# fogg-lab/tissue-model-analysis-tools

Measured on AMD Instinct MI355X. Metric: images/sec (1024x1024 uint16) through compute_branches, higher is better.
Workload: dtype f32; 1 GPU; 256 synthetic 1024x1024 uint16 Z-projections per GPU (256 distinct), inputs pre-resident in HBM (host-pointer entry adds 2 MB/image of H2D), tiled UNet seg (200 patches/image, random-init structured weights) + DMT branch extraction, default_branching_computation.json; images_per_gpu=256, distinct_images=256, patches_per_image=200, rows_gathered=256

## Files before the change

### include/tmat.h

```cpp
#ifndef TMAT_H
#define TMAT_H
#include <stddef.h>
#include <stdint.h>

#ifdef __cplusplus
extern "C" {
#endif

typedef struct tmat_ctx *tmat_handle;

#define TMAT_OK 0
#define TMAT_E_ARG (-1)
#define TMAT_E_HIP (-2)
#define TMAT_E_WEIGHTS (-3)
#define TMAT_E_CAP (-4)

const char *tmat_last_error(void);
int tmat_version(void);

int tmat_create(int device_id, const void *weights_blob, size_t n_bytes, int max_patches, tmat_handle *out);
int tmat_create_plain(int device_id, tmat_handle *out);
void tmat_destroy(tmat_handle h);
int tmat_sync(tmat_handle h);

// ... 288 lines not shown
#define TMAT_PRECISION_F32 0
#define TMAT_PRECISION_BF16X3 1
#define TMAT_PRECISION_BF16X6 2
int tmat_set_precision(tmat_handle h, int mode);

int tmat_set_input_norm(tmat_handle h, int on, double norm_mean, double norm_std);

int tmat_prof_enable(tmat_handle h, int on);
int tmat_prof_read(tmat_handle h, double *ms, int64_t *launches, double *flops, int reset);

int tmat_debug_poison(tmat_handle h, int byte_pattern);

int tmat_debug_held_bytes(tmat_handle h, size_t *device_bytes, size_t *pinned_bytes);

int tmat_debug_filter_stages(tmat_handle h, const uint8_t *mask, int n, int hh, int ww, int use_median, int remove_isolated, uint8_t *median,
                             int32_t *labels, int32_t *stats, uint8_t *skeleton, uint8_t *filtered, int32_t *thin_launches);

int tmat_roi_plan(int hh, int ww, int patch, int n_up, const int *channels, int max_classes, int tiles_cap, int *tiles_per_img,
                  int *n_classes, int *tile_class, int *tile_rank, int *class_count, int *rects, double *mac_planned, double *mac_full);

int tmat_roi_plan_tight(int hh, int ww, int patch, int n_up, const int *channels, int max_classes, int tiles_cap, int *tiles_per_img,
                        int *n_classes, int *tile_class, int *tile_rank, int *class_count, int *rects, double *mac_planned, double *mac_full);
int tmat_roi_plan_exact(int hh, int ww, int patch, int n_up, const int *channels, int max_classes, int tiles_cap, int *tiles_per_img,
                        int *n_classes, int *tile_class, int *tile_rank, int *class_count, int *rects, double *mac_planned, double *mac_full);

int tmat_roi_plan_down(int hh, int ww, int patch, int n_up, const int *up_channels, int n_down, const int *down_channels,
                       unsigned fused_mask, int max_classes, int *n_classes, int *rects, int *needs, double *mac_planned,
                       double *mac_full, double *bytes_planned, double *bytes_full, int *free_tile);

int tmat_roi_sep_tiles(int hh, int ww, int patch, int n_up, const int *up_channels, int n_down, const int *down_channels,
                       unsigned fused_mask, int layer, int k, int cap, int *n_tiles, int *n_full, int *tiles);

int tmat_roi_plan_const(int hh, int ww, int patch, int n_up, const int *up_channels, int n_down, const int *down_channels,
                        unsigned fused_mask, int max_classes, int *n_classes, int *nonconst, int *live, int *rect_live, int *fill,
                        int *stored, double *mac_live, double *bytes_live);
int tmat_roi_sep_tiles_live(int hh, int ww, int patch, int n_up, const int *up_channels, int n_down, const int *down_channels,
                            unsigned fused_mask, int layer, int k, int cap, int *n_tiles, int *n_full, int *tiles);

int tmat_roi_plan_share(int hh, int ww, int patch, int n_up, const int *up_channels, int n_down, const int *down_channels,
                        unsigned fused_mask, int max_classes, int *n_classes, int *inner, int *share, unsigned char *comp,
                        int fill_cap, int *n_fill, int *fills, int tiles_cap, int *neighbours);
int tmat_roi_sep_tiles_share(int hh, int ww, int patch, int n_up, const int *up_channels, int n_down, const int *down_channels,
                             unsigned fused_mask, int layer, int k, int cap, int *n_tiles, int *n_full, int *tiles);
int tmat_roi_plan_share_rect(int hh, int ww, int patch, int n_up, const int *up_channels, int n_down, const int *down_channels,
                             unsigned fused_mask, int max_classes, int *n_classes, int *share, int *n_rects, int *rects,
                             unsigned char *comp, int fill_cap, int *n_fill, int *fills, double *mac_rect, double *bytes_rect, int *info);
int tmat_roi_plan_share_fused_rect(int hh, int ww, int patch, int n_up, const int *up_channels, int n_down, const int *down_channels,
                                   unsigned fused_mask, int max_classes, int *n_classes, int *n_rects, int *rects, unsigned char *comp,
                                   int fill_cap, int *n_fill, int *fills, int *fill_on, double *totals, int *info);
int tmat_roi_down_schedule(int hh, int ww, int patch, int n_up, const int *up_channels, int n_down, const int *down_channels,
                           unsigned fused_mask, int form, int k, int *info, int *n_segs, int *segs, int const_cap, int *n_const,
                           int *const_fills, int copy_cap, int *n_copy, int *copies);
int tmat_debug_share_fill_check(int n_patches, int side, int channels, const int *neighbours, int n_items, const int *items);

int tmat_debug_sep_tiles(tmat_handle h, int cap, int *n, long long *planned, long long *full);
int tmat_debug_down_segs(tmat_handle h, int *max_segs);
int tmat_debug_down_seg_total(tmat_handle h, int *total);

#ifdef __cplusplus
}
#endif
#endif
```

### tissue-model-analysis-tools_amd/csrc/pipeline.cpp

```cpp
#include "../../include/tmat.h"
#include "overlay.h"
#include "png.h"
#include "tmat_ctx.h"
#include "postproc.h"
#include "morph.h"
#include "host_par.h"

#include <algorithm>
#include <atomic>
#include <cmath>
#include <cstring>
#include <chrono>
#include <cstdio>
#include <thread>

namespace tmat {

void launch_lanczos(const uint16_t *img, int n, int H, int W, int h, int w, const int *xi, const float *xc, const int *yi,
                    const float *yc, float *tmp, uint16_t *out, float sat, hipStream_t s);
void launch_rescale01(const uint16_t *x, int n, size_t per, int *mn, int *mx, float *out, hipStream_t s);
void launch_well_zero_f32(float *x, const uint8_t *well, size_t n, hipStream_t s);
void launch_well_seg(const double *pred, const uint8_t *well, uint8_t *seg, size_t n, hipStream_t s);

static int round_half_even(double v) { return (int)std::nearbyint(v); }
// ... 68 lines not shown
    PassBuf &b = c->pass;
    launch_lanczos(imgs_dev, k, b.H, b.W, b.h, b.w, b.xi, b.xc, b.yi, b.yc, b.tmp, b.small, c->input_sat, c->stream);
    launch_rescale01(b.small, k, (size_t)b.h * b.w, b.mn, b.mx, b.x, c->stream);
    int rc = predict_smooth_dev(c, b.x, k, b.h, b.w, b.pred[slot]);
    if (rc) return rc;
    TMAT_HIP(hipMemcpyAsync(b.pred_host[slot], b.pred[slot], (size_t)k * b.h * b.w * sizeof(double), hipMemcpyDeviceToHost, c->stream));
    TMAT_HIP(hipEventRecord(b.done[slot], c->stream));
    return TMAT_OK;
}

static bool use_one_stream()
{
    static const bool one = [] { const char *e = getenv("TMAT_STREAMS"); return !(e && atoi(e) == 2); }();
    return one;
}
static bool tail_on_side_stream()
{
    static const bool side = [] { const char *e = getenv("TMAT_TAIL_STREAM"); return !(e && atoi(e) == 0); }() && use_one_stream();
    return side;
}
static bool pre_on_side_stream(const Ctx *c, const TileGeom &g) { return c->pre_side && tail_on_side_stream() && g.tiles_per_img <= c->max_patches && c->patch_in2; }
static float *patch_in_of(Ctx *c, int slot, const TileGeom &g) { return pre_on_side_stream(c, g) && (slot & 1) ? c->patch_in2 : c->patch_in; }
static int enqueue_pre(Ctx *c, const uint16_t *imgs_dev, int k, int slot, const TileGeom &g, uint16_t *bg_keep = nullptr, const uint8_t *well = nullptr,
                       uint8_t *orig_pic = nullptr)
{
    PassBuf &b = c->pass;
    const bool oversize = g.tiles_per_img > c->max_patches;
    const bool side = pre_on_side_stream(c, g);
    hipStream_t s = side ? c->stream2 : (use_one_stream() || oversize) ? c->stream : c->stream2;
    if (side && c->down_pending[slot]) TMAT_HIP(hipStreamWaitEvent(s, c->ev_down[slot], 0));
    launch_lanczos(imgs_dev, k, b.H, b.W, b.h, b.w, b.xi, b.xc, b.yi, b.yc, b.tmp, b.small, c->input_sat, s);
    if (bg_keep) TMAT_HIP(hipMemcpyAsync(bg_keep, b.small, (size_t)k * b.h * b.w * sizeof(uint16_t), hipMemcpyDeviceToDevice, s));
    launch_rescale01(b.small, k, (size_t)b.h * b.w, b.mn, b.mx, b.x, s);
    if (orig_pic && vis_picture_u16_dev(b.small, k, (size_t)b.h * b.w, b.mn, b.mx, orig_pic, s)) { set_error("analyze (pictures): launch failed"); return TMAT_E_HIP; }
    if (well) launch_well_zero_f32(b.x, well, (size_t)k * b.h * b.w, s);
    if (c->norm_on) launch_norm_f32(b.x, (size_t)k * b.h * b.w, c->norm_mean, c->norm_std, s);
    float *mn = (float *)c->scratch, *mx = mn + k;
    launch_minmax_f32(b.x, k, (size_t)b.h * b.w, mn, mx, s);
    launch_extract_tiles(b.x, mn, k, g, patch_in_of(c, slot, g), s);
    if (c->roi_const != 0 && k <= c->const_cap) TMAT_HIP(hipMemcpyAsync(c->padval[slot], mn, (size_t)k * sizeof(float), hipMemcpyDeviceToDevice, s));
    if (side) TMAT_HIP(hipEventRecord(c->ev_pre[slot], s));
    return TMAT_OK;
}
static int enqueue_down(Ctx *c, int k, int slot, const TileGeom &g)
{
    const bool oversize = g.tiles_per_img > c->max_patches;
    hipStream_t s = (use_one_stream() || oversize) ? c->stream : c->stream2;
    if (pre_on_side_stream(c, g)) TMAT_HIP(hipStreamWaitEvent(s, c->ev_pre[slot], 0));
    if (oversize && tail_on_side_stream() && c->blend_pending[slot ^ 1]) TMAT_HIP(hipStreamWaitEvent(s, c->ev_blend[slot ^ 1], 0));
    float *pin = patch_in_of(c, slot, g);
    const RoiPlan *plan = roi_find(c, g);
    int rc = oversize ? unet_forward_dev(c, pin, k * g.tiles_per_img, c->patch_out, s)
                      : unet_down_dev(c, pin, k * g.tiles_per_img, c->dout[slot], s, plan, c->padval[slot],
                                      roi_down_resolve(c, plan, k, c->padval[slot] != nullptr, true));
    if (rc) return rc;
    TMAT_HIP(hipEventRecord(c->ev_down[slot], s));
    c->down_pending[slot] = true;
    return TMAT_OK;
}
static int enqueue_back(Ctx *c, int k, int slot, const TileGeom &g, const uint8_t *well = nullptr, uint8_t *seg = nullptr)
{
    PassBuf &b = c->pass;
    hipStream_t s = c->stream;
    TMAT_HIP(hipStreamWaitEvent(s, c->ev_down[slot], 0));
    const bool tail_side = tail_on_side_stream();
    if (tail_side && c->blend_pending[slot ^ 1]) TMAT_HIP(hipStreamWaitEvent(s, c->ev_blend[slot ^ 1], 0));
    int rc = g.tiles_per_img > c->max_patches ? TMAT_OK : unet_up_dev(c, c->dout[slot], k * g.tiles_per_img, c->patch_out, s, roi_find(c, g));
    if (rc) return rc;
    if (tail_side) {
        TMAT_HIP(hipEventRecord(c->ev_up[slot], s));
        s = c->stream2;
        TMAT_HIP(hipStreamWaitEvent(s, c->ev_up[slot], 0));
    }
    launch_blend(c->patch_out, c->win1d, k, g, b.pred[slot], s);
    if (tail_side) { TMAT_HIP(hipEventRecord(c->ev_blend[slot], s)); c->blend_pending[slot] = true; }
    const size_t npx = (size_t)k * b.h * b.w;
    if (well) {
        launch_well_seg(b.pred[slot], well, seg, npx, s);
        rc = filter_mask_dev(nullptr, seg, k, b.h, b.w, 1, 1, b.morph_ws, b.filt[slot], b.dist[slot], s);
    } else {
        rc = filter_edt_dev(b.pred[slot], k, b.h, b.w, 1, b.morph_ws, b.filt[slot], b.dist[slot], s);
    }
    if (rc) return TMAT_E_HIP;
    if (thin_on_device(c)) {
        if (thin_count_dev(b.filt[slot], k, b.h, b.w, b.nfg[slot], s)) return TMAT_E_HIP;
        TMAT_HIP(hipMemcpyAsync(b.nfg_host[slot], b.nfg[slot], k * sizeof(int), hipMemcpyDeviceToHost, s));
    } else {
        TMAT_HIP(hipMemcpyAsync(b.filt_host[slot], b.filt[slot], npx, hipMemcpyDeviceToHost, s));
        TMAT_HIP(hipMemcpyAsync(b.dist_host[slot], b.dist[slot], npx * sizeof(double), hipMemcpyDeviceToHost, s));
    }
    TMAT_HIP(hipMemcpyAsync(b.conv_host[slot], morph_done_flags(b.morph_ws, k, b.h, b.w), k * sizeof(int), hipMemcpyDeviceToHost, s));
    TMAT_HIP(hipEventRecord(b.done[slot], s));
    return TMAT_OK;
}

struct GraphParams {
    int fh, fw;
    float t1, t2;
    int smooth, min_len, max_len, remove_isolated;
};

static double now_s() { return std::chrono::duration<double>(std::chrono::steady_clock::now().time_since_epoch()).count(); }
static bool trace_on() { static int t = -1; if (t < 0) { const char *e = getenv("TMAT_TRACE"); t = e && atoi(e) > 0; } return t; }


struct PassJob {
    std::thread th;
// ... 816 lines not shown
```

### tissue-model-analysis-tools_amd/csrc/roi_plan.cpp

```cpp
#include "roi_plan.h"
#include "tmat_internal.h"
#include "../../include/tmat.h"

#include <algorithm>

namespace tmat {

namespace {

struct Iv { int lo, hi; };

Iv clip(Iv v, int R) { return Iv{std::max(v.lo, 0), std::min(v.hi, R)}; }
Iv dilate(Iv v, int d, int R) { return clip(Iv{v.lo - d, v.hi + d}, R); }
Iv hull(Iv a, Iv b) { return Iv{std::min(a.lo, b.lo), std::max(a.hi, b.hi)}; }
Iv halve(Iv v) { return Iv{v.lo >> 1, (v.hi + 1) >> 1}; }
Iv align_cols(Iv v, int R)
{
    int lo = v.lo & ~3, hi = std::min(R, (v.hi + 3) & ~3);
    if (R >= 64 && ((hi - lo) & 7) != 0) {
        if (lo >= 4) lo -= 4;
        else if (hi + 4 <= R) hi += 4;
        else { lo = 0; hi = R; }
    }
    return Iv{lo, hi};
// ... 698 lines not shown
}

static int form_rects(const RoiDownPlan &d, const RoiDownPlan::RectForm *f, int l, int k, RoiRect *out)
{
    if (f) {
        std::copy(f->rects[l][k], f->rects[l][k] + f->n[l][k], out);
        return f->n[l][k];
    }
    out[0] = d.rect_live[l][k];
    return out[0].rh > 0 && out[0].rw > 0 ? 1 : 0;
}

int roi_down_rects(const RoiPlan &p, RoiDownForm form, int l, int k, RoiRect out[4])
{
    const RoiDownPlan &d = p.down;
    switch (roi_down_form(p, form)) {
    case ROI_DOWN_FULL: return 0;
    case ROI_DOWN_REGION: out[0] = d.rect[l][k]; return out[0].rh > 0 && out[0].rw > 0 ? 1 : 0;
    case ROI_DOWN_SHARE_RECT: return form_rects(d, &d.rcomp, l, k, out);
    case ROI_DOWN_SHARE_FUSED_RECT: return form_rects(d, &d.fcomp, l, k, out);
    default: return form_rects(d, nullptr, l, k, out);
    }
}

int roi_down_stem_layer(const RoiPlan &p, RoiDownForm form)
{
    return roi_down_form(p, form) == ROI_DOWN_SHARE_FUSED_RECT ? 6 * p.down.n_down : 4;
}

long long roi_sep_tile_table(const RoiPlan &p, RoiDownForm form, int layer, int k, std::vector<int> &out)
{
    out.clear();
    const RoiDownPlan &d = p.down;
    form = roi_down_form(p, form);
    const int b = layer / 6, kk = layer % 6;
    if (form == ROI_DOWN_FULL || k < 1 || layer < 0 || b >= d.n_down || (kk != 1 && kk != 3) || !((d.fused_mask >> b) & 1u)) return 0;
    const bool share = form >= ROI_DOWN_SHARE;
    const int TW = d.res[layer] / 16, TPP = TW * TW;
    const long long full = (long long)k * p.tiles_per_img * TPP;
    if (full > 0x7fffffffLL || (share && TW > 64)) return 0;
    for (int cl = 0; cl < p.n_classes; cl++) {
        const RoiRect &q = (form == ROI_DOWN_REGION ? d.rect : d.rect_live)[layer][cl];
        const int ty0 = q.y0 / 16, ty1 = (q.y0 + q.rh) / 16, tx0 = q.x0 / 16, tx1 = (q.x0 + q.rw) / 16;
        for (int pt = k * p.class_base[cl]; pt < k * p.class_base[cl + 1]; pt++)
            for (int ty = ty0; ty < ty1; ty++) {
                if (share && !((d.tile_rows[layer][cl] >> ty) & 1ull)) continue;
                for (int tx = tx0; tx < tx1; tx++)
                    if (!share || ((d.tile_cols[layer][cl] >> tx) & 1ull)) out.push_back(pt * TPP + ty * TW + tx);
            }
    }
    return full;
}

void roi_down_segs(const RoiPlan &p, RoiDownForm form, int l, int k, RoiSegs &out)
{
    out = RoiSegs{};
    form = roi_down_form(p, form);
    for (int cl = 0; cl < p.n_classes; cl++) {
        RoiRect q[4];
        const int nq = p.class_count[cl] > 0 ? roi_down_rects(p, form, l, cl, q) : 0;
        for (int i = 0; i < nq; i++) {
            RoiSeg &g = out.s[out.nseg++];
            g.p0 = k * p.class_base[cl]; g.np = k * p.class_count[cl];
            g.y0 = q[i].y0; g.x0 = q[i].x0; g.rh = q[i].rh; g.rw = q[i].rw;
        }
    }
    if (form >= ROI_DOWN_CONST) {
        RoiSeg &g = out.s[out.nseg++];
        g.p0 = k * p.tiles_per_img; g.np = k; g.rh = g.rw = p.down.res[l];
    }
}

void roi_down_const_items(const RoiPlan &p, RoiDownForm form, int l, int k, FillItems &out)
{
    out = FillItems{};
    if (roi_down_form(p, form) < ROI_DOWN_CONST) return;
    for (int cl = 0; cl < p.n_classes; cl++)
        for (int i = 0; i < 4 && p.class_count[cl] > 0; i++) {
            const RoiRect &q = p.down.fill[l][cl][i];
            if (q.rh <= 0 || q.rw <= 0) continue;
            out.it[out.n++] = FillItem{k * p.class_base[cl], k * p.class_count[cl], p.class_count[cl], q.y0, q.x0, q.rh, q.rw};
        }
}

void roi_down_copy_items(const RoiPlan &p, RoiDownForm form, int l, int k, std::vector<ShareItem> &out)
{
    out.clear();
    const RoiDownPlan &d = p.down;
    form = roi_down_form(p, form);
    if (form < ROI_DOWN_SHARE) return;
    auto take = [&](const std::vector<RoiDownPlan::ShareFill> &from) {
        for (const RoiDownPlan::ShareFill &f : from)
            if (f.layer == l) out.push_back(ShareItem{k * p.class_base[f.cls], k * p.class_count[f.cls], f.dir, f.y0, f.x0, f.rh, f.rw});
    };
    take(form == ROI_DOWN_SHARE_FUSED_RECT && d.fused_fill_on[l] ? d.fcomp.fill : d.share_fill);
    if (form >= ROI_DOWN_SHARE_RECT) take(d.rcomp.fill);
}

bool roi_make_plan(int hh, int ww, int ws, int n_up, const int *chan, int max_classes, RoiPlan &out)
{
    out = RoiPlan();
    if (hh < 1 || ww < 1 || ws < 1 || n_up < 1 || n_up > ROI_MAX_UP || !chan || (ws % (4 << n_up)) != 0) return false;
    max_classes = std::min(max_classes, ROI_MAX_CLASSES);
    const TileGeom g = make_geom(hh, ww, ws);
    out.hh = hh; out.ww = ww; out.ws = ws; out.n_up = n_up;
    out.tiles_per_img = g.tiles_per_img;
// ... 183 lines not shown
    const bool args_ok = n_classes && rects && needs && mac_planned && mac_full && bytes_planned && bytes_full && free_tile;
    if (int rc = down_plan_for("tmat_roi_plan_down", args_ok, hh, ww, patch, n_up, up_channels, n_down, down_channels, fused_mask, max_classes, p)) return rc;
    *n_classes = p.n_classes;
    const RoiDownPlan &d = p.down;
    for (int l = 0; l < d.n_layers; l++) {
        for (int k = 0; k < max_classes; k++) {
            const size_t at = ((size_t)l * max_classes + k) * 4;
            put_rect(rects + at, d.rect[l][k], k < p.n_classes);
            put_rect(needs + at, d.need[l][k], k < p.n_classes);
        }
        mac_planned[l] = d.mac_planned[l]; mac_full[l] = d.mac_full[l];
        bytes_planned[l] = d.bytes_planned[l]; bytes_full[l] = d.bytes_full[l];
    }
    for (int b = 0; b < d.n_down; b++) free_tile[b] = d.free_tile[b] ? 1 : 0;
    return TMAT_OK;
}

static int sep_tiles_export(RoiDownForm form, int hh, int ww, int patch, int n_up, const int *up_channels, int n_down, const int *down_channels,
                            unsigned fused_mask, int layer, int k, int cap, int *n_tiles, int *n_full, int *tiles)
{
    RoiPlan p;
    if (int rc = down_plan_for("tmat_roi_sep_tiles", n_tiles && n_full && k >= 1, hh, ww, patch, n_up, up_channels, n_down, down_channels, fused_mask,
                               ROI_MAX_CLASSES, p)) return rc;
    std::vector<int> tab;
    const long long full = roi_sep_tile_table(p, form, layer, k, tab);
    if (full <= 0) { set_error("tmat_roi_sep_tiles: not a fused separable layer of the plan"); return TMAT_E_ARG; }
    *n_full = (int)full;
    *n_tiles = (int)tab.size();
    if (tiles) {
        if ((int)tab.size() > cap) { set_error("tmat_roi_sep_tiles: cap too small"); return TMAT_E_ARG; }
        std::copy(tab.begin(), tab.end(), tiles);
    }
    return TMAT_OK;
}

extern "C" int tmat_roi_sep_tiles(int hh, int ww, int patch, int n_up, const int *up_channels, int n_down, const int *down_channels,
                                  unsigned fused_mask, int layer, int k, int cap, int *n_tiles, int *n_full, int *tiles)
{
    return sep_tiles_export(ROI_DOWN_REGION, hh, ww, patch, n_up, up_channels, n_down, down_channels, fused_mask, layer, k, cap, n_tiles, n_full, tiles);
}

extern "C" int tmat_roi_sep_tiles_live(int hh, int ww, int patch, int n_up, const int *up_channels, int n_down, const int *down_channels,
                                       unsigned fused_mask, int layer, int k, int cap, int *n_tiles, int *n_full, int *tiles)
{
    return sep_tiles_export(ROI_DOWN_CONST, hh, ww, patch, n_up, up_channels, n_down, down_channels, fused_mask, layer, k, cap, n_tiles, n_full, tiles);
}

extern "C" int tmat_roi_sep_tiles_share(int hh, int ww, int patch, int n_up, const int *up_channels, int n_down, const int *down_channels,
                                        unsigned fused_mask, int layer, int k, int cap, int *n_tiles, int *n_full, int *tiles)
{
    return sep_tiles_export(ROI_DOWN_SHARE, hh, ww, patch, n_up, up_channels, n_down, down_channels, fused_mask, layer, k, cap, n_tiles, n_full, tiles);
}

extern "C" int tmat_roi_plan_const(int hh, int ww, int patch, int n_up, const int *up_channels, int n_down, const int *down_channels,
                                   unsigned fused_mask, int max_classes, int *n_classes, int *nonconst, int *live, int *rect_live, int *fill,
                                   int *stored, double *mac_live, double *bytes_live)
{
    RoiPlan p;
    const bool args_ok = n_classes && nonconst && live && rect_live && fill && stored && mac_live && bytes_live;
    if (int rc = down_plan_for("tmat_roi_plan_const", args_ok, hh, ww, patch, n_up, up_channels, n_down, down_channels, fused_mask, max_classes, p)) return rc;
    *n_classes = p.n_classes;
    const RoiDownPlan &d = p.down;
    for (int l = 0; l < d.n_layers; l++) {
        for (int k = 0; k < max_classes; k++) {
            const bool in = k < p.n_classes;
            const size_t at = ((size_t)l * max_classes + k) * 4;
            put_rect(nonconst + at, d.nonconst[l][k], in);
            put_rect(live + at, d.live[l][k], in);
            put_rect(rect_live + at, d.rect_live[l][k], in);
            for (int i = 0; i < 4; i++) put_rect(fill + (at + i) * 4, d.fill[l][k][i], in);
        }
        stored[l] = d.stored[l] ? 1 : 0;
        mac_live[l] = d.mac_live[l]; bytes_live[l] = d.bytes_live[l];
    }
    return TMAT_OK;
}

extern "C" int tmat_roi_plan_share(int hh, int ww, int patch, int n_up, const int *up_channels, int n_down, const int *down_channels,
                                   unsigned fused_mask, int max_classes, int *n_classes, int *inner, int *share, unsigned char *comp,
                                   int fill_cap, int *n_fill, int *fills, int tiles_cap, int *neighbours)
{
    RoiPlan p;
    const bool args_ok = n_classes && inner && share && comp && n_fill && fills && neighbours && fill_cap >= 0;
    if (int rc = down_plan_for("tmat_roi_plan_share", args_ok, hh, ww, patch, n_up, up_channels, n_down, down_channels, fused_mask, max_classes, p)) return rc;
    const RoiDownPlan &d = p.down;
    if (p.tiles_per_img > tiles_cap || (int)d.nbr.size() != 3 * p.tiles_per_img) { set_error("tmat_roi_plan_share: tiles_cap too small"); return TMAT_E_ARG; }
    *n_classes = p.n_classes;
    for (int l = 0; l < d.n_layers; l++) {
        for (int k = 0; k < max_classes; k++) {
            const size_t at = ((size_t)l * max_classes + k) * 4;
            put_rect(inner + at, d.inner[l][k], k < p.n_classes);
            for (int i = 0; i < 4; i++) share[at + i] = k < p.n_classes ? d.share[l][k][i] : 0;
        }
        put_masks(p, d.comp, l, max_classes, comp);
    }
    std::copy(d.nbr.begin(), d.nbr.end(), neighbours);
    return put_fill_list("tmat_roi_plan_share", d.share_fill, fill_cap, n_fill, fills);
}

extern "C" int tmat_roi_plan_share_rect(int hh, int ww, int patch, int n_up, const int *up_channels, int n_down, const int *down_channels,
                                        unsigned fused_mask, int max_classes, int *n_classes, int *share, int *n_rects, int *rects,
                                        unsigned char *comp, int fill_cap, int *n_fill, int *fills, double *mac_rect, double *bytes_rect, int *info)
{
    RoiPlan p;
    const bool args_ok = n_classes && share && n_rects && rects && comp && n_fill && fills && mac_rect && bytes_rect && info && fill_cap >= 0;
    if (int rc = down_plan_for("tmat_roi_plan_share_rect", args_ok, hh, ww, patch, n_up, up_channels, n_down, down_channels, fused_mask, max_classes, p)) return rc;
// ... 86 lines not shown
```

### tissue-model-analysis-tools_amd/csrc/roi_plan.h

```cpp
#pragma once
#include <vector>

namespace tmat {

constexpr int ROI_MAX_CLASSES = 16;
constexpr int ROI_MAX_UP = 5;
constexpr int ROI_MAX_LAYERS = 3 * ROI_MAX_UP + 1;
constexpr int ROI_MAX_DOWN = 4;
constexpr int ROI_MAX_DOWN_LAYERS = 6 * ROI_MAX_DOWN + 4;

struct RoiRect { int y0, x0, rh, rw; };
struct RoiSegs;
struct FillItems;
struct ShareItem;

constexpr unsigned ROI_EXACT_KEEP_TIGHT = 0u;

struct RoiDownPlan {
    struct ShareFill { int layer, cls, dir, y0, x0, rh, rw; };
    int n_down = 0, n_layers = 0;
    unsigned fused_mask = 0;
    int res[ROI_MAX_DOWN_LAYERS] = {};
    RoiRect need[ROI_MAX_DOWN_LAYERS][ROI_MAX_CLASSES] = {}, rect[ROI_MAX_DOWN_LAYERS][ROI_MAX_CLASSES] = {};
    double mac_planned[ROI_MAX_DOWN_LAYERS] = {}, mac_full[ROI_MAX_DOWN_LAYERS] = {};
    double bytes_planned[ROI_MAX_DOWN_LAYERS] = {}, bytes_full[ROI_MAX_DOWN_LAYERS] = {};
    bool free_tile[ROI_MAX_DOWN] = {};

    RoiRect nonconst[ROI_MAX_DOWN_LAYERS][ROI_MAX_CLASSES] = {}, live[ROI_MAX_DOWN_LAYERS][ROI_MAX_CLASSES] = {};
    RoiRect rect_live[ROI_MAX_DOWN_LAYERS][ROI_MAX_CLASSES] = {};
    RoiRect fill[ROI_MAX_DOWN_LAYERS][ROI_MAX_CLASSES][4] = {};
    bool stored[ROI_MAX_DOWN_LAYERS] = {};
    double mac_live[ROI_MAX_DOWN_LAYERS] = {}, bytes_live[ROI_MAX_DOWN_LAYERS] = {};

    bool share_any = false;
    RoiRect inner[ROI_MAX_DOWN_LAYERS][ROI_MAX_CLASSES] = {};
    int share[ROI_MAX_DOWN_LAYERS][ROI_MAX_CLASSES][4] = {};
    unsigned long long tile_rows[ROI_MAX_DOWN_LAYERS][ROI_MAX_CLASSES] = {}, tile_cols[ROI_MAX_DOWN_LAYERS][ROI_MAX_CLASSES] = {};
    std::vector<unsigned char> comp;
    std::vector<ShareFill> share_fill;
    std::vector<int> nbr;

    struct RectForm {
        bool any = false;
        int n[ROI_MAX_DOWN_LAYERS][ROI_MAX_CLASSES] = {};
        RoiRect rects[ROI_MAX_DOWN_LAYERS][ROI_MAX_CLASSES][4] = {};
        std::vector<unsigned char> mask;
        std::vector<ShareFill> fill;
        double mac[ROI_MAX_DOWN_LAYERS] = {}, bytes[ROI_MAX_DOWN_LAYERS] = {}, px[ROI_MAX_DOWN_LAYERS] = {};
        int segs = 0;
    };
    int rshare[ROI_MAX_DOWN_LAYERS][ROI_MAX_CLASSES][4] = {};
    RectForm rcomp;
    bool fused_fill_on[ROI_MAX_DOWN_LAYERS] = {};
    RectForm fcomp;
    double px_live[ROI_MAX_DOWN_LAYERS] = {};
    double copy_old[ROI_MAX_DOWN_LAYERS] = {}, copy_new[ROI_MAX_DOWN_LAYERS] = {};
};

enum RoiDownForm { ROI_DOWN_FULL, ROI_DOWN_REGION, ROI_DOWN_CONST, ROI_DOWN_SHARE, ROI_DOWN_SHARE_RECT, ROI_DOWN_SHARE_FUSED_RECT };

constexpr unsigned ROI_SHARE_LEVELS = 3u;
constexpr unsigned ROI_SHARE_RECT_LEVELS = 4u;
constexpr unsigned ROI_SHARE_FUSED_RECT_LEVELS = 3u;

struct RoiPlan {
    int hh = 0, ww = 0, ws = 0, n_up = 0;
    int tiles_per_img = 0;
    int n_classes = 0;
    int n_layers = 0;
    int class_base[ROI_MAX_CLASSES + 1] = {};
    int class_count[ROI_MAX_CLASSES] = {};
    std::vector<int> tile_class, tile_rank;
    int res[ROI_MAX_LAYERS] = {};
    RoiRect rect[ROI_MAX_LAYERS][ROI_MAX_CLASSES] = {};
    RoiRect rect_tight[ROI_MAX_LAYERS][ROI_MAX_CLASSES] = {};
    RoiRect rect_exact[ROI_MAX_LAYERS][ROI_MAX_CLASSES] = {};
    bool tight = false, exact = false;
    const RoiRect *up_rects(int l) const { return tight ? (exact ? rect_exact[l] : rect_tight[l]) : rect[l]; }
    RoiRect read[ROI_MAX_CLASSES] = {};
    double mac_planned[ROI_MAX_LAYERS] = {}, mac_full[ROI_MAX_LAYERS] = {};
    double mac_planned_tight[ROI_MAX_LAYERS] = {};
    double mac_planned_exact[ROI_MAX_LAYERS] = {};
    RoiDownPlan down;
};

bool roi_make_plan(int hh, int ww, int ws, int n_up, const int *chan, int max_classes, RoiPlan &out);
bool roi_plan_down(RoiPlan &p, int n_down, const int *chan, unsigned fused_mask);
void roi_plan_share(RoiPlan &p);

RoiDownForm roi_down_form(const RoiPlan &p, RoiDownForm want);
int roi_down_rects(const RoiPlan &p, RoiDownForm form, int l, int k, RoiRect out[4]);
int roi_down_stem_layer(const RoiPlan &p, RoiDownForm form);
long long roi_sep_tile_table(const RoiPlan &p, RoiDownForm form, int layer, int k, std::vector<int> &out);
void roi_down_segs(const RoiPlan &p, RoiDownForm form, int l, int k, RoiSegs &out);
void roi_down_const_items(const RoiPlan &p, RoiDownForm form, int l, int k, FillItems &out);
void roi_down_copy_items(const RoiPlan &p, RoiDownForm form, int l, int k, std::vector<ShareItem> &out);
void roi_share_neighbours(const RoiPlan &p, int k, std::vector<int> &out);

}
```

### tissue-model-analysis-tools_amd/csrc/sepconv_ws_kernels.hip

```cpp
#include "dev_guard.h"
#include "tmat_internal.h"
#include "../../include/tmat.h"

#include <cstdio>
#include <cstdlib>
#include <type_traits>

namespace tmat {

typedef float f32x16 __attribute__((ext_vector_type(16)));
typedef __attribute__((address_space(3))) void lds_void_t;
typedef __bf16 bf16x8 __attribute__((ext_vector_type(8)));

constexpr int WS_A = 256 * 32, WS_X = 1024, WS_B = 128 * 32, WS_NHP = 13, WS_HP = WS_NHP * 256;
constexpr int WS_A0 = 0, WS_A1 = WS_A + WS_X, WS_B0 = WS_A1 + WS_A, WS_B1 = WS_B0 + WS_B, WS_H = WS_B1 + WS_B;
constexpr int WS_TOTAL = WS_H + 4 * WS_HP;
static_assert(WS_TOTAL * 4 <= 160 * 1024, "LDS budget");
constexpr int WS_WPITCH = 22, WS_WP = 21 * WS_WPITCH, WS_NWP = (WS_WP + 63) / 64, WS_WIN = WS_TOTAL, WS_TOTAL_STEM = WS_WIN + 4 * WS_NWP * 64;
static_assert(WS_TOTAL_STEM * 4 <= 160 * 1024, "LDS budget (stem form)");
static_assert(8 * 9 * 128 <= WS_A + WS_X, "exchange buffer fits an A stage + gap");

struct WsArgs {
    const float *in;
    int N, H, W, Cin, Cout;
    const float *dw9;
    const float *pwk;
    const float *scale, *shift;
    int relu_out;
    float *out;
    const float *resid;
    float *strip_h, *strip_v, *corner;
    const float *stem_w, *stem_scale, *stem_shift;
};

__device__ __forceinline__ int ws_pixmap_y(int r) { return ((r >= 4 && r < 12) || (r >= 16 && r < 20) || r >= 28) ? 1 : 0; }
__device__ __forceinline__ int ws_pixmap_x(int r) { return r < 4 ? r : r < 12 ? r - 4 : r < 16 ? r - 8 : r < 20 ? r - 8 : r < 28 ? r - 12 : r - 16; }

#define WS_BAR() { asm volatile("" ::: "memory"); __builtin_amdgcn_s_barrier(); asm volatile("" ::: "memory"); }
#define WS_PIN() __builtin_amdgcn_sched_barrier(0);
#ifdef WS_DIAG
__device__ long long ws_diag[256 * 12 * 8];
#define WS_STAMP(k) { const long long now_ = (long long)__builtin_readcyclecounter(); dsum[k] += now_ - dlast; dlast = now_; }
#define WS_DIAG_DECL long long dsum[8] = {0, 0, 0, 0, 0, 0, 0, 0}, dlast = (long long)__builtin_readcyclecounter();
#define WS_DIAG_FLUSH() if (lane == 0 && blockIdx.x < 256) { for (int k = 0; k < 8; k++) ws_diag[((size_t)blockIdx.x * 12 + wave) * 8 + k] = dsum[k]; }
__device__ long long ws_tl[12 * 2 * 14];
#define WS_TL(k) if (lane == 0 && blockIdx.x == 0 && (s == 13 || s == 15)) ws_tl[(wave * 2 + (s == 15)) * 14 + (k)] = (long long)__builtin_readcyclecounter();
#else
#define WS_TL(k)
#define WS_STAMP(k)
#define WS_DIAG_DECL
#define WS_DIAG_FLUSH()
#endif

__device__ __forceinline__ int ws_tab_read(int mt, RoiNone) { return mt; }
__device__ __forceinline__ int ws_tab_read(int mt, const int *tab)
{
    return *((const __attribute__((address_space(4))) int *)(unsigned long long)tab + mt);
}

template <bool RELU_IN, bool POOL, int PREC = 0, bool STEM = false, bool ROI = false>
__global__ __launch_bounds__(768, 3) void sepconv_ws_kernel(WsArgs a, int nMt, int nNt, int G, std::conditional_t<ROI, const int *, RoiNone> tab)
{
    static_assert(!ROI || PREC == 0, "ROI: f32 path only");
    __shared__ __attribute__((aligned(16))) float smem[STEM ? WS_TOTAL_STEM : WS_TOTAL];

    const int b = blockIdx.x;
    const int bp = (b & 7) * (G >> 3) + (b >> 3);
    const long long P = (long long)nMt * nNt;
    const int j0 = (int)(P * bp / G), j1 = (int)(P * (bp + 1) / G);
    if (j0 >= j1) return;

    const int t = threadIdx.x;
    const int lane = t & 63, wave = __builtin_amdgcn_readfirstlane(t >> 6);
    const int TW = a.W >> 4, TPP = (a.H >> 4) * TW;
    const int Cin = a.Cin;
    const int nchunks = Cin >> 5;
    const int total = (j1 - j0) * nchunks;
    constexpr unsigned OOB = 0x80000000u;

    if (STEM) {
        for (int e = t; e < 9 * Cin; e += 768) smem[WS_A + e] = a.dw9[e];
        asm volatile("s_waitcnt vmcnt(0) lgkmcnt(0)" ::: "memory");
        WS_BAR()
    }
    if (wave >= 8) {
        const int p = wave - 8;
#ifndef WS_PRODUCER_PRIO
#define WS_PRODUCER_PRIO 3
#endif
        __builtin_amdgcn_s_setprio(WS_PRODUCER_PRIO);
        const int oy = (p >> 1) * 8, ox = (p & 1) * 8;
        float *Hp = smem + WS_H + p * WS_HP;
        const int q = lane & 7, xl = lane >> 3;
        const int Xt = ox + xl;
        const int r0 = Xt < 4 ? Xt : Xt < 8 ? Xt + 8 : Xt + 12;
        const int r1 = Xt < 8 ? Xt + 4 : Xt < 12 ? Xt + 8 : Xt + 16;
        const int aoff0 = ((oy >> 1) * 32 + r0) * 32 + ((q ^ ((r0 >> 1) & 7)) * 4);
        const int aoff1 = ((oy >> 1) * 32 + r1) * 32 + ((q ^ ((r1 >> 1) & 7)) * 4);
        const int hoff = xl * 32 + q * 4;
        const unsigned bvo0 = (unsigned)((32 * p + (lane >> 3)) * Cin * 4 + (((lane & 7) ^ (lane >> 4)) * 16));
        const unsigned bvo1 = (unsigned)((32 * p + 8 + (lane >> 3)) * Cin * 4 + (((lane & 7) ^ (4 + (lane >> 4))) * 16));
        const unsigned bvo_p = (unsigned)((64 * (p & 1) + (lane >> 2)) * Cin * 2 + (((lane & 3) ^ ((lane >> 4) & 3)) * 16));

        unsigned rel[WS_NHP], hv[WS_NHP];
        unsigned m_top = 0, m_bot = 0, m_left = 0, m_right = 0, m_inv = 0;
#pragma unroll
        for (int i = 0; i < WS_NHP; i++) {
            const int hp = 8 * i + (lane >> 3);
            const int hy = hp / 10, hx = hp - hy * 10;
            rel[i] = (unsigned)((hy * a.W + hx) * Cin + (lane & 7) * 4) * 4u;
            m_top |= (unsigned)(hy == 0) << i; m_bot |= (unsigned)(hy == 9) << i;
            m_left |= (unsigned)(hx == 0) << i; m_right |= (unsigned)(hx == 9) << i;
            m_inv |= (unsigned)(hp >= 100) << i;
        }
        unsigned badw = 0;
        unsigned w_top = 0, w_bot = 0, w_left = 0, w_right = 0, w_inv = 0;
        unsigned badm = 0;
        float *Wp = smem + WS_WIN + p * (WS_NWP * 64);
        if (STEM) {
#pragma unroll
            for (int i = 0; i < WS_NWP; i++) {
                const int e = 64 * i + lane;
                const int wy = e / WS_WPITCH, wx = e - wy * WS_WPITCH;
                w_top |= (unsigned)(wy < 2) << i; w_bot |= (unsigned)(wy >= 18) << i;
                w_left |= (unsigned)(wx < 2) << i; w_right |= (unsigned)(wx >= 18) << i;
                w_inv |= (unsigned)(e >= WS_WP) << i;
            }
        }
        const float *hA = a.in;
        int tnext = ws_tab_read(j0 / nNt, tab);
        auto tile_setup = [&](int jj) {
            const int mt = ROI ? tnext : jj / nNt;
            if (ROI) tnext = ws_tab_read((jj + 1 < j1 ? jj + 1 : jj) / nNt, tab);
            const int n = mt / TPP, tr = mt - n * TPP;
            const int Y0 = (tr / TW) * 16 + oy - 1, X0 = (tr % TW) * 16 + ox - 1;
            const unsigned bad = m_inv | (Y0 < 0 ? m_top : 0u) | (Y0 + 9 >= a.H ? m_bot : 0u) | (X0 < 0 ? m_left : 0u) | (X0 + 9 >= a.W ? m_right : 0u);
            if (STEM) {
                hA = a.in + ((long)n * a.H * a.W * 4 + (long)(2 * Y0) * (2 * a.W) + 2 * X0);
                badw = w_inv | (Y0 < 0 ? w_top : 0u) | (Y0 + 9 >= a.H ? w_bot : 0u) | (X0 < 0 ? w_left : 0u) | (X0 + 9 >= a.W ? w_right : 0u);
                badm = bad;
            } else {
                hA = a.in + ((long)n * a.H * a.W + (long)Y0 * a.W + X0) * Cin;
#pragma unroll
                for (int i = 0; i < WS_NHP; i++) hv[i] = ((bad >> i) & 1u) ? OOB : rel[i];
            }
        };
        int hj = j0, hc = 0;
        auto issue_halo = [&]() {
            const __amdgpu_buffer_rsrc_t rsA = __builtin_amdgcn_make_buffer_rsrc((void *)hA, 0, 0x7fffffff, 0x00020000);
            if (STEM) {
                if (hc == 0) {
                    int lane_o = lane;
                    asm volatile("" : "+v"(lane_o));
#pragma unroll
                    for (int i = 0; i < WS_NWP; i++) {
                        const int e = 64 * i + lane_o;
                        const int wy = e / WS_WPITCH, wx = e - wy * WS_WPITCH;
                        const unsigned relw = (unsigned)(wy * 2 * a.W + wx) * 4u;
                        __builtin_amdgcn_raw_ptr_buffer_load_lds(rsA, (lds_void_t *)(Wp + i * 64), 4, ((badw >> i) & 1u) ? OOB : relw, 0, 0, 0);
                    }
                }
            } else {
#pragma unroll
                for (int i = 0; i < WS_NHP; i++)
                    __builtin_amdgcn_raw_ptr_buffer_load_lds(rsA, (lds_void_t *)(Hp + i * 256), 16, hv[i], hc * 128, 0, 0);
            }
            if (++hc == nchunks) { hc = 0; hj++; }
        };
        WS_DIAG_DECL
        int pj = j0, pc = 0;
        float4 wt[9];
        float4 sw[9], ssc, ssh;
        const __amdgpu_buffer_rsrc_t rsT = __builtin_amdgcn_make_buffer_rsrc((void *)a.dw9, 0, 0x7fffffff, 0x00020000);
        int cur_pc = 0;
        auto load_taps = [&]() {
            if (!STEM) {
#pragma unroll
                for (int tp = 0; tp < 9; tp++)
                    wt[tp] = __builtin_bit_cast(float4, __builtin_amdgcn_raw_buffer_load_b128(rsT, q * 16, (tp * Cin + pc * 32) * 4, 0));
            }
            if (STEM) {
                cur_pc = pc;
                const __amdgpu_buffer_rsrc_t rsW = __builtin_amdgcn_make_buffer_rsrc((void *)a.stem_w, 0, 0x7fffffff, 0x00020000);
                const __amdgpu_buffer_rsrc_t rsC = __builtin_amdgcn_make_buffer_rsrc((void *)a.stem_scale, 0, 0x7fffffff, 0x00020000);
                const __amdgpu_buffer_rsrc_t rsH = __builtin_amdgcn_make_buffer_rsrc((void *)a.stem_shift, 0, 0x7fffffff, 0x00020000);
#pragma unroll
                for (int tp = 0; tp < 9; tp++)
                    sw[tp] = __builtin_bit_cast(float4, __builtin_amdgcn_raw_buffer_load_b128(rsW, q * 16, (tp * Cin + pc * 32) * 4, 0));
// ... 149 lines not shown
#ifdef WS_VAR_SLEEP
            __builtin_amdgcn_s_sleep(WS_VAR_SLEEP);
#endif
#ifdef WS_VAR_FETCHPRIO
            __builtin_amdgcn_s_setprio(WS_VAR_FETCHPRIO);
#endif
            if (s + 1 < total) fetch((s + 1) & 1);
            WS_STAMP(3)
            WS_TL(1)
            WS_BAR()
#ifdef WS_VAR_FETCHPRIO
            __builtin_amdgcn_s_setprio(WS_PRODUCER_PRIO);
#endif
            WS_STAMP(4)
            WS_TL(2)
            if (s + 1 < total) compute((s + 1) & 1);
            WS_STAMP(5)
            WS_TL(3)
            if (++cc == nchunks) {
                cc = 0;
                if (POOL) WS_BAR()
            }
            WS_BAR()
            WS_STAMP(6)
            WS_TL(4)
        }
#ifdef WS_DIAG
        dsum[7] = total;
#endif
        WS_DIAG_FLUSH()
        return;
    }

    const int r = lane & 31, h = lane >> 5;
    const int key = (r >> 1) & 7;
    const int aoffc = (32 * wave + r) * 32, boffc = r * 32;

    f32x16 acc[4];
#pragma unroll
    for (int jn = 0; jn < 4; jn++)
#pragma unroll
        for (int e = 0; e < 16; e++) acc[jn][e] = 0.f;

    float scv[4], shv[4];
    auto load_scale_shift = [&](int jj) {
        const int n0 = (jj % nNt) * 128;
#pragma unroll
        for (int jn = 0; jn < 4; jn++) { scv[jn] = a.scale[n0 + jn * 32 + r]; shv[jn] = a.shift[n0 + jn * 32 + r]; }
    };
    const int CoutB = a.Cout * 4;
    const float relu_lo = a.relu_out ? 0.f : -__builtin_inff();
    const unsigned vo_pool = (unsigned)(4 * h * a.Cout + r) * 4u;
    float rv[4][4];
    int ctile = ws_tab_read(j0 / nNt, tab);
    auto load_resid = [&](int jj) {
        const int mc = jj / nNt, nt = jj - mc * nNt;
        const int mt = ROI ? ctile : mc;
        const int n = mt / TPP, tr = mt - n * TPP;
        const int ty = tr / TW, tx = tr - ty * TW;
        const __amdgpu_buffer_rsrc_t rsR = __builtin_amdgcn_make_buffer_rsrc(
            (void *)(a.resid + (((size_t)n * (a.H >> 1) + ty * 8 + wave) * (a.W >> 1) + tx * 8) * a.Cout + nt * 128), 0, 0x7fffffff, 0x00020000);
        if (wave < 7) {
#pragma unroll
            for (int jn = 0; jn < 4; jn++)
#pragma unroll
                for (int qq = 0; qq < 4; qq++)
                    rv[jn][qq] = __builtin_bit_cast(float, __builtin_amdgcn_raw_buffer_load_b32(rsR, vo_pool, qq * CoutB + jn * 128, 0));
        }
    };

    unsigned vo_t[4];
#pragma unroll
    for (int i = 0; i < 4; i++) {
        const int pix = 8 * i + (lane >> 3);
        vo_t[i] = (unsigned)(((pix >> 4) * a.W + (pix & 15)) * a.Cout + (lane & 7) * 4) * 4u;
    }
    auto store_tile = [&](int jj, float *xw) {
        const int mc = jj / nNt, nt = jj - mc * nNt;
        const int mt = ROI ? ctile : mc;
        const int n = mt / TPP, tr = mt - n * TPP;
        const int ty0 = (tr / TW) * 16, tx0 = (tr % TW) * 16;
        const __amdgpu_buffer_rsrc_t rsO = __builtin_amdgcn_make_buffer_rsrc(
            (void *)(a.out + ((size_t)n * a.H * a.W + (size_t)(ty0 + 2 * wave) * a.W + tx0) * a.Cout + nt * 128), 0, 0x7fffffff, 0x00020000);
        float *xl = xw + r;
        const float *xr = xw + lane * 4;
#pragma unroll
        for (int jn = 0; jn < 4; jn++) {
            const float sc = scv[jn], sh = shv[jn];
#pragma unroll
            for (int e = 0; e < 16; e++) {
                const int yy = (e >= 4 && e < 12) ? 1 - h : h;
                xl[(yy * 16 + e) * 32] = fmaxf(fmaf(acc[jn][e], sc, sh), relu_lo);
                acc[jn][e] = 0.f;
            }
            float4 o[4];
#pragma unroll
            for (int i = 0; i < 4; i++) o[i] = *reinterpret_cast<const float4 *>(xr + i * 256);
#pragma unroll
            for (int i = 0; i < 4; i++)
                __builtin_amdgcn_raw_buffer_store_b128(__builtin_bit_cast(__attribute__((ext_vector_type(4))) unsigned, o[i]), rsO, vo_t[i], jn * 128, 0);
        }
    };

    int tl_s = -1;
    auto store_tile_pool = [&](int jj, float *xch) {
#ifdef WS_DIAG
        const int s = tl_s;
#endif
        constexpr int NW = 8, XC = 128;
        const int mc = jj / nNt, nt = jj - mc * nNt;
        const int mt = ROI ? ctile : mc;
        const int n = mt / TPP, tr = mt - n * TPP;
        const int ty = tr / TW, tx = tr - ty * TW;
        const int n0 = nt * 128;
        const size_t T = (size_t)n * TPP + tr;
        float hm[4][4], vs[4];
        constexpr float NEG = -__builtin_inff();
        const __amdgpu_buffer_rsrc_t rsP = __builtin_amdgcn_make_buffer_rsrc(
            (void *)(a.out + (((size_t)n * (a.H >> 1) + ty * NW + wave) * (a.W >> 1) + tx * 8) * a.Cout + n0), 0, 0x7fffffff, 0x00020000);
        const __amdgpu_buffer_rsrc_t rsSH = __builtin_amdgcn_make_buffer_rsrc((void *)(a.strip_h + T * 8 * a.Cout + n0), 0, 0x7fffffff, 0x00020000);
        const __amdgpu_buffer_rsrc_t rsSV = __builtin_amdgcn_make_buffer_rsrc((void *)(a.strip_v + (T * NW + wave) * a.Cout + n0), 0, 0x7fffffff, 0x00020000);
        const __amdgpu_buffer_rsrc_t rsCO = __builtin_amdgcn_make_buffer_rsrc((void *)(a.corner + T * a.Cout + n0), 0, 0x7fffffff, 0x00020000);
#pragma unroll
        for (int jn = 0; jn < 4; jn++) {
            const float sc = scv[jn], sh = shv[jn];
            float v[16];
            if (a.relu_out) {
#pragma unroll
                for (int e = 0; e < 16; e++) v[e] = fmaxf(fmaf(acc[jn][e], sc, sh), 0.f);
            } else {
#pragma unroll
                for (int e = 0; e < 16; e++) v[e] = fmaf(acc[jn][e], sc, sh);
            }
#pragma unroll
            for (int e = 0; e < 16; e++) acc[jn][e] = 0.f;
#ifndef WS_POOL_SHUFFLE
            const float v8 = v[8], o8 = __shfl_xor(v8, 32);
            float y0[9], m01[9];
#pragma unroll
            for (int k = 0; k < 8; k++) {
                float A = v[k], B = v[8 + k];
                asm volatile("s_nop 1\n\tv_permlane32_swap_b32 %0, %1\n\ts_nop 1" : "+v"(A), "+v"(B));
                m01[k] = fmaxf(A, B);
                y0[k] = ((h != 0) != (k >= 4)) ? B : A;
            }
            y0[8] = h ? NEG : o8;
            m01[8] = h ? NEG : fmaxf(o8, v8);
#else
            float y0[9], y1[9];
#pragma unroll
            for (int k = 0; k < 8; k++) {
                const float own = h ? v[8 + k] : v[k];
                const float oth = __shfl_xor(h ? v[k] : v[8 + k], 32);
// ... 107 lines not shown
                bf16x8 ahi, alo;
#pragma unroll
                for (int j = 0; j < 8; j++) {
                    const __bf16 q = (__bf16)xs[j];
                    ahi[j] = q;
                    alo[j] = (__bf16)(xs[j] - (float)q);
                }
#pragma unroll
                for (int jn = 0; jn < 4; jn++) {
                    acc[jn] = __builtin_amdgcn_mfma_f32_32x32x16_bf16(alo, wq[0][jn], acc[jn], 0, 0, 0);
                    acc[jn] = __builtin_amdgcn_mfma_f32_32x32x16_bf16(ahi, wq[1][jn], acc[jn], 0, 0, 0);
                    acc[jn] = __builtin_amdgcn_mfma_f32_32x32x16_bf16(ahi, wq[0][jn], acc[jn], 0, 0, 0);
                }
                WS_PIN()
            }
        } else {
        WS_READ_A(0)
        WS_READ_A(1)
        WS_PIN()
#ifdef WS_DIAG
        asm volatile("s_waitcnt lgkmcnt(0)" ::: "memory");
        WS_TL(1)
        WS_PIN()
#endif
        WS_MM(0)
        WS_PIN()
        WS_TL(2)
        WS_READ_A(2)
        WS_READ_B(2, Bs)
        WS_PIN()
        WS_MM(1)
        WS_PIN()
        WS_TL(3)
        WS_READ_A(3)
        WS_READ_B(3, Bs)
        WS_PIN()
        WS_MM(2)
        WS_PIN()
        WS_TL(4)
        WS_MM(3)
        WS_PIN()
        }
        WS_TL(5)
        WS_STAMP(1)
        WS_BAR()
        WS_STAMP(2)
        WS_TL(6)
        if (++cc == nchunks) {
            cc = 0;
            tl_s = s;
            if (POOL) store_tile_pool(cj, smem + (stage ? WS_A : 0));
            else store_tile(cj, smem + (stage ? WS_A1 : WS_A0) + wave * 1024);
            cj++;
            if (ROI && s + 1 < total) ctile = ws_tab_read(cj / nNt, tab);
        }
        WS_PIN()
        if (s + 1 < total) {
            if (cc == 0) load_scale_shift(cj);
            if (POOL && nchunks > 1 && cc == nchunks - 1) load_resid(cj);
        }
        WS_PIN()
        if (s + 1 < total) {
            if (PREC == 0) {
                const float *Bn = smem + (stage ? WS_B0 : WS_B1) + boffc;
                WS_READ_B(0, Bn)
                WS_READ_B(1, Bn)
            } else {
                const float *Bn = smem + (stage ? WS_B0 : WS_B1);
                WS_READ_BP(0, Bn)
            }
        }
        WS_PIN()
        WS_STAMP(3)
        WS_TL(7)
        WS_BAR()
        WS_STAMP(4)
        WS_TL(8)
    }
#undef WS_READ_A
#undef WS_READ_B
#undef WS_READ_BP
#undef WS_MM
#ifdef WS_DIAG
    dsum[7] = total;
#endif
    WS_DIAG_FLUSH()
}

bool sepconv_ws_supported(int H, int W, int Cin, int Cout)
{
    return H % 16 == 0 && W % 16 == 0 && Cin % 32 == 0 && Cout % 128 == 0 &&
           (long long)H * W * Cin * 4 < 0x7fffffffLL && (long long)Cout * Cin * 4 < 0x7fffffffLL;
}

static bool ws_tiles_ok(const int *tiles, int n_tiles, int N, int H, int W, int prec)
{
    return !tiles || (prec == 0 && n_tiles > 0 && (long long)n_tiles <= (long long)N * (H / 16) * (W / 16));
}

static int ws_cus()
{
    static int n_cu = 0;
    if (!n_cu) {
        int dev = 0;
        hipDeviceProp_t prop;
        if (hipGetDevice(&dev) != hipSuccess || hipGetDeviceProperties(&prop, dev) != hipSuccess || prop.multiProcessorCount < 8) n_cu = 256;
        else n_cu = prop.multiProcessorCount;
    }
    return n_cu;
}

template <bool POOL>
static void launch_ws_any(const WsArgs &a, int relu_in, int prec, hipStream_t s, const int *tiles = nullptr, int n_tiles = 0)
{
    const int nMt = tiles ? n_tiles : a.N * (a.H / 16) * (a.W / 16), nNt = a.Cout / 128;
    const int G = (ws_cus() / 8) * 8;
    if (prec == 1) {
        if (relu_in) hipLaunchKernelGGL((sepconv_ws_kernel<true, POOL, 1>), dim3(G), dim3(768), 0, s, a, nMt, nNt, G, RoiNone{});
        else hipLaunchKernelGGL((sepconv_ws_kernel<false, POOL, 1>), dim3(G), dim3(768), 0, s, a, nMt, nNt, G, RoiNone{});
    } else if (tiles) {
        if (relu_in) hipLaunchKernelGGL((sepconv_ws_kernel<true, POOL, 0, false, true>), dim3(G), dim3(768), 0, s, a, nMt, nNt, G, tiles);
        else hipLaunchKernelGGL((sepconv_ws_kernel<false, POOL, 0, false, true>), dim3(G), dim3(768), 0, s, a, nMt, nNt, G, tiles);
    } else if (relu_in) hipLaunchKernelGGL((sepconv_ws_kernel<true, POOL>), dim3(G), dim3(768), 0, s, a, nMt, nNt, G, RoiNone{});
    else hipLaunchKernelGGL((sepconv_ws_kernel<false, POOL>), dim3(G), dim3(768), 0, s, a, nMt, nNt, G, RoiNone{});
#ifdef WS_DIAG
    {
        static long long hbuf[256 * 12 * 8];
        hipStreamSynchronize(s);
        hipMemcpyFromSymbol(hbuf, HIP_SYMBOL(ws_diag), sizeof(hbuf));
        double cs[8] = {0}, ps[8] = {0};
        const int nb = G < 256 ? G : 256;
        for (int b = 0; b < nb; b++)
            for (int w = 0; w < 12; w++)
                for (int k = 0; k < 8; k++) (w < 8 ? cs : ps)[k] += (double)hbuf[((size_t)b * 12 + w) * 8 + k];
        const double cst = cs[7], pst = ps[7];
        fprintf(stderr, "[wsdiag] H %d Cin %d Cout %d pool %d | consumer per step: top %.0f mfma %.0f barX %.0f epilogue %.0f barY %.0f | producer per step: issue %.0f vmcnt0 %.0f rows %.0f barX %.0f compute %.0f barY %.0f | steps/wave %.0f\n",
                a.H, a.Cin, a.Cout, (int)POOL, cs[0] / cst, cs[1] / cst, cs[2] / cst, cs[3] / cst, cs[4] / cst,
                ps[0] / pst, ps[1] / pst, ps[2] / pst, (ps[3] + ps[4]) / pst, ps[5] / pst, ps[6] / pst, cst / (nb * 8.0));
        static long long tl[12 * 2 * 14];
        hipMemcpyFromSymbol(tl, HIP_SYMBOL(ws_tl), sizeof(tl));
        for (int st = 0; st < 2; st++) {
            long long t0 = tl[st * 14];
            for (int w = 0; w < 12; w++) if (tl[(w * 2 + st) * 14] < t0) t0 = tl[(w * 2 + st) * 14];
            for (int w = 0; w < 12; w++) {
                fprintf(stderr, "[wstl] step %d wave %2d:", st ? 15 : 13, w);
                for (int k = 0; k < (w < 8 ? 13 : 5); k++) fprintf(stderr, " %6lld", tl[(w * 2 + st) * 14 + k] - t0);
                fprintf(stderr, "\n");
            }
        }
    }
#endif
}

bool launch_sepconv_ws(const float *in, int N, int H, int W, int Cin, int relu_in, const float *dw9, const float *pwk, int Cout,
                       const float *scale, const float *shift, int relu_out, float *out, hipStream_t s, int prec, const int *tiles, int n_tiles)
{
    if (!sepconv_ws_supported(H, W, Cin, Cout) || N <= 0 || (long long)N * (H / 16) * (W / 16) * (Cout / 128) > 0x3fffffffLL ||
        !ws_tiles_ok(tiles, n_tiles, N, H, W, prec)) {
        set_error("launch_sepconv_ws: unsupported shape");
        return false;
    }
    WsArgs a{in, N, H, W, Cin, Cout, dw9, pwk, scale, shift, relu_out, out, nullptr, nullptr, nullptr, nullptr, nullptr, nullptr, nullptr};
    launch_ws_any<false>(a, relu_in, prec, s, tiles, n_tiles);
    return true;
}

bool launch_sepconv_ws_stem(const float *x, int N, int H, int W, int Cin, const float *stem_w, const float *stem_scale, const float *stem_shift,
                            const float *dw9, const float *pwk, int Cout, const float *scale, const float *shift, int relu_out, float *out,
                            hipStream_t s, const int *tiles, int n_tiles)
{
    if (!sepconv_ws_supported(H, W, Cin, Cout) || N <= 0 || (long long)N * (H / 16) * (W / 16) * (Cout / 128) > 0x3fffffffLL || 9 * Cin > WS_X ||
        !ws_tiles_ok(tiles, n_tiles, N, H, W, 0)) {
        set_error("launch_sepconv_ws_stem: unsupported shape");
        return false;
    }
    WsArgs a{x, N, H, W, Cin, Cout, dw9, pwk, scale, shift, relu_out, out, nullptr, nullptr, nullptr, nullptr, stem_w, stem_scale, stem_shift};
    const int nMt = tiles ? n_tiles : N * (H / 16) * (W / 16), nNt = Cout / 128;
    const int G = (ws_cus() / 8) * 8;
    if (tiles) hipLaunchKernelGGL((sepconv_ws_kernel<false, false, 0, true, true>), dim3(G), dim3(768), 0, s, a, nMt, nNt, G, tiles);
    else hipLaunchKernelGGL((sepconv_ws_kernel<false, false, 0, true>), dim3(G), dim3(768), 0, s, a, nMt, nNt, G, RoiNone{});
    return true;
}

template <bool ROI>
__global__ __launch_bounds__(256) void pool_fix_add_kernel(float *__restrict__ out, const float *__restrict__ strip_h, const float *__restrict__ strip_v,
                                                           const float *__restrict__ corner, const float *__restrict__ resid, int Hp, int Wp, int C,
                                                           int c4shift, int total, int PR, std::conditional_t<ROI, RoiSegs, RoiNone> roi)
{
    const int n = blockIdx.y;
    const int e = blockIdx.x * 256 + threadIdx.x;
    const int cq = e & ((1 << c4shift) - 1);
    const int TH = Hp / PR, TW = Wp >> 3;
    auto finish = [&](int ty, int pl, int tx, int ql) {
    const size_t o = (((size_t)n * Hp + ty * PR + pl) * Wp + tx * 8 + ql) * C + cq * 4;
    float4 m = *reinterpret_cast<const float4 *>(out + o);
    auto take = [&](const float *src) {
        const float4 v = *reinterpret_cast<const float4 *>(src + cq * 4);
        m.x = fmaxf(m.x, v.x); m.y = fmaxf(m.y, v.y); m.z = fmaxf(m.z, v.z); m.w = fmaxf(m.w, v.w);
    };
    const bool below = pl == PR - 1 && ty + 1 < TH, right = ql == 7 && tx + 1 < TW;
    if (below) take(strip_h + ((((size_t)n * TH + ty + 1) * TW + tx) * 8 + ql) * C);
    if (right) take(strip_v + ((((size_t)n * TH + ty) * TW + tx + 1) * PR + pl) * C);
    if (below && right) take(corner + (((size_t)n * TH + ty + 1) * TW + tx + 1) * C);
    const float4 rv = *reinterpret_cast<const float4 *>(resid + o);
    m.x = m.x + rv.x; m.y = m.y + rv.y; m.z = m.z + rv.z; m.w = m.w + rv.w;
    *reinterpret_cast<float4 *>(out + o) = m;
    };
    if (!ROI) {
        if (e >= total) return;
        const int bp = e >> c4shift;
        const int NB = 8 + PR - 1;
        const int tile = bp / NB, k = bp - tile * NB;
        const int ty = tile / TW, tx = tile - ty * TW;
        finish(ty, k < 8 ? PR - 1 : k - 8, tx, k < 8 ? k : 7);
        return;
    }
    RoiBox2 rb{};
    if (!roi_box_of(roi, n, rb)) return;
    const bool two_r = rb.y2 != rb.y0, two_c = rb.x2 != rb.x0;
    const int nr0 = rb.y1 - rb.y0, nr = rb.rows(), nc0 = rb.x1 - rb.x0, nc = rb.cols();
    const int br0 = rb.y1 / PR - rb.y0 / PR, br = br0 + (two_r ? rb.y3 / PR - rb.y2 / PR : 0);
    const int bc0 = (rb.x1 >> 3) - (rb.x0 >> 3), bc = bc0 + (two_c ? (rb.x3 >> 3) - (rb.x2 >> 3) : 0);
    const int nA = br * nc, nAB = nA + nr * bc;
    const int step = (int)(gridDim.x * 256) >> c4shift;
    for (int g = e >> c4shift; g < nAB; g += step) {
        int y, x;
        if (g < nA) {
            const int j = g / nc, i = g - j * nc;
            y = (j < br0 ? rb.y0 / PR + j : rb.y2 / PR + (j - br0)) * PR + PR - 1;
            x = i < nc0 ? rb.x0 + i : rb.x2 + (i - nc0);
        } else {
            const int j = (g - nA) / bc, i = (g - nA) - j * bc;
// ... 53 lines not shown
```

### tissue-model-analysis-tools_amd/csrc/tmat_api.cpp

```cpp
#include "../../include/tmat.h"
#include "tmat_ctx.h"
#include "png.h"

#include <algorithm>
#include <cmath>
#include <cstring>
#include <mutex>

namespace tmat {

static std::mutex g_err_mu;
static std::string g_err;
void set_error(const std::string &msg)
{
    std::lock_guard<std::mutex> lk(g_err_mu);
    g_err = msg;
}
bool hip_ok(hipError_t e, const char *what)
{
    if (e == hipSuccess) return true;
    set_error(std::string(what) + ": " + hipGetErrorString(e));
    return false;
}

// ... 198 lines not shown
        cin = u.cout;
    }
    if (!need(m, "final.w", w) || !need(m, "final.b", b)) return false;
    {
        const int C = cin;
        if ((int)w.count != 9 * C || C % 4) { set_error("weights: final conv must be 3x3xCx1"); return false; }
        const std::vector<float> sub = subpixel_weights(std::vector<float>(w.data, w.data + w.count), C, 1);
        std::vector<float> q((size_t)16 * C);
        for (int cg = 0; cg < C / 4; cg++)
            for (int ct = 0; ct < 16; ct++)
                for (int e = 0; e < 4; e++) q[((size_t)cg * 16 + ct) * 4 + e] = sub[(size_t)ct * C + cg * 4 + e];
        if (!upload(c, q, &c->final_w)) return false;
    }
    c->final_b = b.data[0];
    c->f_last = cin;
    if (c->down.size() != c->up.size() - 1 || c->down.empty()) { set_error("weights: unexpected block structure"); return false; }
    int P = c->patch;
    if (P % (8 << c->down.size()) || P <= 0) { set_error("weights: patch size must be divisible by 2^(blocks+1)"); return false; }
    return true;
}

static void prof_begin(Ctx *c, double flops, hipStream_t st)
{
    if (!c->prof_on) return;
    hipEvent_t e0, e1;
    if (c->ev_pool.size() >= 2) { e0 = c->ev_pool.back(); c->ev_pool.pop_back(); e1 = c->ev_pool.back(); c->ev_pool.pop_back(); }
    else { hipEventCreate(&e0); hipEventCreate(&e1); }
    hipEventRecord(e0, st);
    c->ev_open.push_back({e0, e1, flops});
}
static void prof_end(Ctx *c, hipStream_t st)
{
    if (!c->prof_on) return;
    hipEventRecord(c->ev_open.back().e1, st);
}

static bool conv(Ctx *c, ConvArgs a, hipStream_t st, const RoiSegs *roi = nullptr)
{
    bool dom = a.ksize == 3 && a.Cout % 128 == 0 && !a.relu_in;
    if (dom) {
        const double px = roi ? (double)roi->pixels() : (double)a.N * a.h * a.w;
        prof_begin(c, 2.0 * px * 9.0 * a.Cin * a.Cout, st);
    }
    if (c->precision != TMAT_PRECISION_F32) {
        auto &mp = c->wsplit[c->precision];
        auto it = mp.find(a.W);
        if (it != mp.end()) { a.W = it->second; a.prec = c->precision; }
    }
    bool ok = launch_conv(a, st, roi);
    if (dom) prof_end(c, st);
    return ok;
}

static const RoiTileTab *roi_tile_tab(RoiEntry *e, int layer, int k, RoiDownForm form)
{
    form = roi_down_form(e->plan, std::min(form, ROI_DOWN_SHARE));
    for (const RoiTileTab &t : e->tabs) if (t.layer == layer && t.k == k && t.form == form) return &t;
    std::vector<int> ids;
    RoiTileTab t;
    t.layer = layer; t.k = k; t.form = form;
    t.full = roi_sep_tile_table(e->plan, form, layer, k, ids);
    t.n_rep = (long long)ids.size(); t.full_rep = t.full;
    if (t.full <= 0 || ids.empty()) { set_error("roi_tile_tab: no tile table for this layer"); return nullptr; }
    if (form >= ROI_DOWN_CONST) {
        const int TW = e->plan.down.res[layer] / 16, TPP = TW * TW;
        if (t.full + (long long)k * TPP > 0x7fffffffLL) { set_error("roi_tile_tab: too many tiles"); return nullptr; }
        for (int id = (int)t.full; id < (int)t.full + k * TPP; id++) ids.push_back(id);
        t.full += (long long)k * TPP;
    }
    t.n = (int)ids.size();
    if ((long long)ids.size() < t.full) {
        if (!hip_ok(hipMalloc((void **)&t.dev, ids.size() * sizeof(int)), "hipMalloc(tile table)")) return nullptr;
        if (!hip_ok(hipMemcpy(t.dev, ids.data(), ids.size() * sizeof(int), hipMemcpyHostToDevice), "hipMemcpy(tile table)")) { hipFree(t.dev); return nullptr; }
    }
    e->tabs.push_back(t);
    return &e->tabs.back();
}

static const RoiShareTab *roi_share_tab(RoiEntry *e, int k, RoiDownForm form)
{
    for (const RoiShareTab &t : e->shares) if (t.k == k && t.form == form) return &t;
    const RoiPlan &p = e->plan;
    RoiShareTab t;
    t.k = k; t.form = form;
    roi_share_neighbours(p, k, t.nbr);
    for (int l = 0; l < p.down.n_layers; l++) {
        RoiShareTab::Layer sl;
        sl.layer = l;
        roi_down_copy_items(p, form, l, k, sl.items);
        if (!sl.items.empty()) t.layers.push_back(sl);
    }
    auto up = [](const void *src, size_t bytes, void **dev) {
        return bytes == 0 || (hip_ok(hipMalloc(dev, bytes), "hipMalloc(share table)") &&
                              hip_ok(hipMemcpy(*dev, src, bytes, hipMemcpyHostToDevice), "hipMemcpy(share table)"));
    };
    bool ok = up(t.nbr.data(), t.nbr.size() * sizeof(int), (void **)&t.nbr_dev);
    for (RoiShareTab::Layer &l : t.layers) ok = ok && up(l.items.data(), l.items.size() * sizeof(ShareItem), (void **)&l.dev);
    if (!ok) {
        if (t.nbr_dev) hipFree(t.nbr_dev);
        for (RoiShareTab::Layer &l : t.layers) if (l.dev) hipFree(l.dev);
        return nullptr;
    }
    e->shares.push_back(t);
    return &e->shares.back();
}

static bool down_block_ws(const Ctx *c, size_t bi)
{
    const DownBlock &d = c->down[bi];
    const int H = (c->patch / 2) >> bi;
    return c->fused_sep && sepconv_ws_supported(H, H, d.cin, d.cout) && sepconv_ws_supported(H, H, d.cout, d.cout) &&
           ((d.cout / 4) & (d.cout / 4 - 1)) == 0;
}

static RoiSegs roi_segs(const RoiPlan &p, int l, int k)
{
    const RoiRect *rects = p.up_rects(l);
    RoiSegs r{};
    for (int cl = 0; cl < p.n_classes; cl++) {
        const RoiRect &q = rects[cl];
        if (q.rh <= 0 || q.rw <= 0 || p.class_count[cl] <= 0) continue;
        RoiSeg &g = r.s[r.nseg++];
        g.p0 = k * p.class_base[cl]; g.np = k * p.class_count[cl];
        g.y0 = q.y0; g.x0 = q.x0; g.rh = q.rh; g.rw = q.rw;
    }
    return r;
}

static RoiEntry *roi_entry_of(const Ctx *c, const RoiPlan *plan)
{
    for (RoiEntry *e : c->roi_cache) if (&e->plan == plan) return e;
    return nullptr;
}

RoiDownForm roi_down_resolve(const Ctx *c, const RoiPlan *plan, int kimg, bool have_padval, bool by_default)
{
    if (!plan || plan->n_classes <= 0 || plan->down.n_down != (int)c->down.size() || kimg < 1) return ROI_DOWN_FULL;
    auto on = [&](int sw) { return by_default ? sw != 0 : sw == 1; };
    RoiDownForm want = ROI_DOWN_REGION;
    if (on(c->roi_const) && have_padval && c->roi_down && c->precision == TMAT_PRECISION_F32 && kimg <= c->const_cap &&
        plan->n_classes < ROI_MAX_CLASSES) want = ROI_DOWN_CONST;
    if (want == ROI_DOWN_CONST && on(c->roi_share) && (c->roi_down & 2u) && roi_entry_of(c, plan)) want = ROI_DOWN_SHARE;
    if (want == ROI_DOWN_SHARE && on(c->roi_share_rect) && (c->roi_down & 1u)) want = ROI_DOWN_SHARE_RECT;
    if (want == ROI_DOWN_SHARE_RECT && on(c->roi_share_fused_rect)) want = ROI_DOWN_SHARE_FUSED_RECT;
    return roi_down_form(*plan, want);
}

int unet_down_dev(Ctx *c, const float *X, int n, float *dout, hipStream_t s, const RoiPlan *plan, const float *padval, RoiDownForm form)
{
    if (n <= 0) return TMAT_OK;
    if (n > c->max_patches) { set_error("unet_down_dev: n > max_patches"); return TMAT_E_ARG; }
    if (!plan || n % plan->tiles_per_img != 0) form = ROI_DOWN_FULL;
    if (form >= ROI_DOWN_CONST && !padval) { set_error("unet_down_dev: the constant-ring form needs the pad values"); return TMAT_E_ARG; }
    const bool roi_b = form != ROI_DOWN_FULL && (c->roi_down & 1u);
    const int kimg = form != ROI_DOWN_FULL ? n / plan->tiles_per_img : 0;
    const int n_own = n;
    if (form >= ROI_DOWN_CONST) {
        launch_const_patches(padval, kimg, c->patch * c->patch, const_cast<float *>(X) + (size_t)n * c->patch * c->patch, s);
        n += kimg;
    }
    c->sep_tiles.clear();
    c->down_segs = c->down_seg_total = 0;
    RoiSegs sg{};
    auto segs_of = [&](int l) -> const RoiSegs * {
        if (!roi_b) return nullptr;
        roi_down_segs(*plan, form, l, kimg, sg);
        c->down_segs = std::max(c->down_segs, sg.nseg);
        c->down_seg_total += sg.nseg;
        return &sg;
    };
    auto segs = [&](size_t bi, int k) -> const RoiSegs * { return segs_of(6 * (int)bi + k); };
    const int LD = 6 * (int)c->down.size();
    RoiEntry *ent = form != ROI_DOWN_FULL && (c->roi_down & 2u) ? roi_entry_of(c, plan) : nullptr;
    bool tab_ok = true;
    const RoiShareTab *shr = nullptr;
    if (form >= ROI_DOWN_SHARE && !(ent && (shr = roi_share_tab(ent, kimg, form)))) return TMAT_E_HIP;
    auto copies = [&](float *t, int l, int C) -> bool {
        if (form < ROI_DOWN_CONST) return true;
        FillItems f;
        roi_down_const_items(*plan, form, l, kimg, f);
        if (!launch_const_fill(t, n_own, n, plan->down.res[l], C, f, s)) return false;
        if (!shr) return true;
        for (const RoiShareTab::Layer &sl : shr->layers)
            if (sl.layer == l && !launch_share_fill(t, n_own, plan->down.res[l], C, shr->nbr.data(), shr->nbr_dev, sl.items.data(), sl.dev, (int)sl.items.size(), s))
                return false;
        return true;
    };
    auto tiles = [&](size_t bi, int k, int H, bool f32) -> RoiTileTab {
        RoiTileTab t;
        t.full = t.n = n * (H / 16) * (H / 16);
        t.full_rep = t.n_rep = (long long)n_own * (H / 16) * (H / 16);
        if (ent && f32) {
            if (const RoiTileTab *made = roi_tile_tab(ent, 6 * (int)bi + k, kimg, form)) t = *made;
            else tab_ok = false;
        }
        c->sep_tiles.push_back({t.dev ? t.n_rep : t.full_rep, t.full_rep});
        return t;
    };
    const int P = c->patch;
    float *b0 = c->buf[0], *b1 = c->buf[1], *b2 = c->buf[2], *b3 = c->buf[3];
    const int di = dout == c->dout[1] ? 1 : 0;
    c->dout_relu_ok[di] = false;
    const bool stem_in_sep = c->stem_fused && !c->down.empty() && down_block_ws(c, 0) && c->down[0].cin == c->f0 &&
                             !(c->precision == TMAT_PRECISION_BF16X3 && c->sep_bf16);
    if (stem_in_sep) {
        launch_stem_even(X, n, P, P, c->stem_w, c->f0, c->stem_scale, c->stem_shift, b0, s, segs_of(form == ROI_DOWN_FULL ? 4 : roi_down_stem_layer(*plan, form)));
        if (!copies(b0, LD, c->f0)) return TMAT_E_ARG;
    } else launch_stem(X, n, P, P, c->stem_w, c->f0, c->stem_scale, c->stem_shift, b0, s);
    int H = P / 2;
    for (size_t bi = 0; bi < c->down.size(); bi++) {
        auto &d = c->down[bi];
        if (down_block_ws(c, bi)) {
            const float *pw0 = d.pw[0], *pw1 = d.pw[1];
            int sprec = 0;
            if (c->precision == TMAT_PRECISION_BF16X3 && c->sep_bf16) {
                auto &mp = c->wsplit[c->precision];
                auto i0 = mp.find(d.pw[0]), i1 = mp.find(d.pw[1]);
                if (i0 != mp.end() && i1 != mp.end()) { pw0 = i0->second; pw1 = i1->second; sprec = 1; }
            }
            const bool stem_here = bi == 0 && stem_in_sep;
            const RoiTileTab t0 = tiles(bi, 1, H, sprec == 0), t1 = tiles(bi, 3, H, sprec == 0);
            if (!tab_ok) return TMAT_E_HIP;
            if (stem_here) {
                if (!launch_sepconv_ws_stem(X, n, H, H, d.cin, c->stem_w, c->stem_scale, c->stem_shift, d.dw[0], pw0, d.cout, d.scale[0], d.shift[0], 1, b2, s,
                                            t0.dev, t0.n)) return TMAT_E_ARG;
            } else if (!launch_sepconv_ws(b0, n, H, H, d.cin, bi > 0, d.dw[0], pw0, d.cout, d.scale[0], d.shift[0], 1, b2, s, sprec, t0.dev, t0.n)) return TMAT_E_ARG;
            if (!copies(b2, 6 * (int)bi + 1, d.cout)) return TMAT_E_ARG;
            ConvArgs r{};
            r.in = b0; r.N = n; r.h = H; r.w = H; r.Cin = d.cin; r.ksize = 1; r.stride = 2; r.W = d.res_w; r.Cout = d.cout;
            r.scale = nullptr; r.shift = d.res_b; r.out = b1;
            if (stem_here) { r.h = H / 2; r.w = H / 2; r.stride = 1; }
            if (!conv(c, r, s, segs(bi, 4)) || !copies(b1, 6 * (int)bi + 4, d.cout)) return TMAT_E_ARG;
            float *nxt = bi + 1 == c->down.size() ? dout : b0;
            if (c->fused_pool) {
                if (!launch_sepconv_pool_ws(b2, n, H, H, d.cout, 0, d.dw[1], pw1, d.cout, d.scale[1], d.shift[1], 0, b3, b1, nxt, s, sprec, segs(bi, 5),
                                            t1.dev, t1.n)) return TMAT_E_ARG;
            } else {
                if (!launch_sepconv_ws(b2, n, H, H, d.cout, 0, d.dw[1], pw1, d.cout, d.scale[1], d.shift[1], 0, b3, s, sprec, t1.dev, t1.n)) return TMAT_E_ARG;
                launch_maxpool_add(b3, n, H, H, d.cout, b1, nxt, s, nullptr, segs(bi, 5));
            }
            if (!copies(nxt, 6 * (int)bi + 5, d.cout)) return TMAT_E_ARG;
            H /= 2;
            continue;
        }
        const int l0 = 6 * (int)bi;
        launch_dwconv(b0, n, H, H, d.cin, 1, d.dw[0], b1, s, segs(bi, 0));
        if (!copies(b1, l0, d.cin)) return TMAT_E_ARG;
        ConvArgs a{};
        a.in = b1; a.N = n; a.h = H; a.w = H; a.Cin = d.cin; a.relu_in = 0; a.ksize = 1; a.stride = 1;
        a.W = d.pw[0]; a.Cout = d.cout; a.scale = d.scale[0]; a.shift = d.shift[0]; a.resid = nullptr; a.rs = 0;
        a.relu_out = 1; a.out = b2;
        if (!conv(c, a, s, segs(bi, 1)) || !copies(b2, l0 + 1, d.cout)) return TMAT_E_ARG;
        launch_dwconv(b2, n, H, H, d.cout, 0, d.dw[1], b3, s, segs(bi, 2));
        if (!copies(b3, l0 + 2, d.cout)) return TMAT_E_ARG;
        a.in = b3; a.Cin = d.cout; a.W = d.pw[1]; a.scale = d.scale[1]; a.shift = d.shift[1]; a.relu_out = 0; a.out = b2;
        if (!conv(c, a, s, segs(bi, 3)) || !copies(b2, l0 + 3, d.cout)) return TMAT_E_ARG;
        ConvArgs r{};
        r.in = b0; r.N = n; r.h = H; r.w = H; r.Cin = d.cin; r.ksize = 1; r.stride = 2; r.W = d.res_w; r.Cout = d.cout;
        r.scale = nullptr; r.shift = d.res_b; r.out = b1;
        if (!conv(c, r, s, segs(bi, 4)) || !copies(b1, l0 + 4, d.cout)) return TMAT_E_ARG;
        const bool last = bi + 1 == c->down.size();
        float *dr = (last && c->relu_copy && dout == c->dout[di]) ? c->dout_relu[di] : nullptr;
        launch_maxpool_add(b2, n, H, H, d.cout, b1, last ? dout : b0, s, dr, segs(bi, 5));
        if (!copies(last ? dout : b0, l0 + 5, d.cout) || (dr && !copies(dr, l0 + 5, d.cout))) return TMAT_E_ARG;
        if (dr) c->dout_relu_ok[di] = true;
        H /= 2;
    }
    TMAT_HIP(hipGetLastError());
    return TMAT_OK;
}


const RoiPlan *roi_find(const Ctx *c, const TileGeom &g)
{
    if (!g.order) return nullptr;
    for (const RoiEntry *e : c->roi_cache) if (e->order == g.order) return &e->plan;
    return nullptr;
}

// ... 73 lines not shown
        S = so; S_act = so_act; so_idx = so_idx == 2 ? 3 : 2;
        Hs = Hl; up = 1;
    }
    launch_final(S, n, Hs, Hs, c->f_last, c->final_w, c->final_b, Y, s, segs(3 * (int)c->up.size()));
    TMAT_HIP(hipGetLastError());
    return TMAT_OK;
}

int unet_forward_dev(Ctx *c, const float *X, int n, float *Y, hipStream_t s)
{
    const size_t pp = (size_t)c->patch * c->patch;
    for (int i0 = 0; i0 < n; i0 += c->max_patches) {
        const int k = std::min(c->max_patches, n - i0);
        int rc = unet_down_dev(c, X + (size_t)i0 * pp, k, c->dout[0], s);
        if (rc) return rc;
        rc = unet_up_dev(c, c->dout[0], k, Y + (size_t)i0 * pp, s);
        if (rc) return rc;
    }
    return TMAT_OK;
}

int ensure_patch_io(Ctx *c, int n_patches)
{
    if (n_patches <= c->patch_cap) return TMAT_OK;
    TMAT_HIP(hipStreamSynchronize(c->stream));
    TMAT_HIP(hipStreamSynchronize(c->stream2));
    for (float *p : {c->patch_in, c->patch_in2, c->patch_out}) c->ws.release(p);
    c->patch_in = c->patch_in2 = c->patch_out = nullptr;
    c->patch_cap = 0;
    const size_t bytes = (size_t)c->patch * c->patch * n_patches * sizeof(float);
    c->patch_in = (float *)c->ws.dev(bytes + (size_t)c->patch * c->patch * c->const_cap * sizeof(float), "hipMalloc(patch_in)");
    c->patch_out = (float *)c->ws.dev(bytes, "hipMalloc(patch_out)");
    if (!c->patch_in || !c->patch_out) return TMAT_E_HIP;
    c->patch_cap = n_patches;
    return TMAT_OK;
}

int predict_smooth_dev(Ctx *c, float *x_dev, int n, int hh, int ww, double *pred_dev)
{
    if (c->norm_on) launch_norm_f32(x_dev, (size_t)n * hh * ww, c->norm_mean, c->norm_std, c->stream);
    const int P = c->patch;
    TileGeom g = make_geom(hh, ww, P);
    const RoiPlan *plan = roi_attach(c, g);
    const int per_pass = std::max(1, c->max_patches / g.tiles_per_img);
    { int rc = ensure_patch_io(c, per_pass * g.tiles_per_img); if (rc) return rc; }
    size_t need_pv = (size_t)std::min(n, per_pass) * 2 * sizeof(float);
    if (need_pv > c->scratch_bytes) { set_error("predict_smooth: scratch too small"); return TMAT_E_ARG; }
    float *mn = (float *)c->scratch, *mx = mn + std::min(n, per_pass);
    for (int i0 = 0; i0 < n; i0 += per_pass) {
        int k = std::min(per_pass, n - i0);
        const float *xi = x_dev + (size_t)i0 * hh * ww;
        launch_minmax_f32(xi, k, (size_t)hh * ww, mn, mx, c->stream);
        launch_extract_tiles(xi, mn, k, g, c->patch_in, c->stream);
        int rc = plan ? unet_down_dev(c, c->patch_in, k * g.tiles_per_img, c->dout[0], c->stream, plan, mn, roi_down_resolve(c, plan, k, true, false))
                      : unet_forward_dev(c, c->patch_in, k * g.tiles_per_img, c->patch_out, c->stream);
        if (!rc && plan) rc = unet_up_dev(c, c->dout[0], k * g.tiles_per_img, c->patch_out, c->stream, plan);
        if (rc) return rc;
        launch_blend(c->patch_out, c->win1d, k, g, pred_dev + (size_t)i0 * hh * ww, c->stream);
    }
    TMAT_HIP(hipGetLastError());
    return TMAT_OK;
}

}

using namespace tmat;

extern "C" {

const char *tmat_last_error(void)
{
    static thread_local std::string copy;
    std::lock_guard<std::mutex> lk(g_err_mu);
    copy = g_err;
    return copy.c_str();
}
int tmat_version(void) { return 0x000100; }

int tmat_create_plain(int device_id, tmat_handle *out)
{
    if (!out) { set_error("tmat_create_plain: null argument"); return TMAT_E_ARG; }
    *out = nullptr;
    int ndev = 0;
    if (hipGetDeviceCount(&ndev) != hipSuccess || ndev <= 0) {
        set_error("tmat_create_plain: no HIP device available (libtmat_hip has no CPU fallback)");
        return TMAT_E_HIP;
    }
    if (device_id < 0 || device_id >= ndev) { set_error("tmat_create_plain: bad device id"); return TMAT_E_ARG; }
    TMAT_HIP(hipSetDevice(device_id));
    Ctx *c = new Ctx();
    c->device = device_id;
    if (!hip_ok(hipStreamCreate(&c->stream), "hipStreamCreate")) { tmat_destroy((tmat_handle)c); return TMAT_E_HIP; }
    { const int rc = resnet_precision_from_env(c); if (rc) { tmat_destroy((tmat_handle)c); return rc; } }
    *out = (tmat_handle)c;
    return TMAT_OK;
}

int tmat_create(int device_id, const void *weights_blob, size_t n_bytes, int max_patches, tmat_handle *out)
{
    if (!out || !weights_blob) { set_error("tmat_create: null argument"); return TMAT_E_ARG; }
    *out = nullptr;
    int ndev = 0;
    if (hipGetDeviceCount(&ndev) != hipSuccess || ndev <= 0) {
        set_error("tmat_create: no HIP device available (libtmat_hip has no CPU fallback)");
        return TMAT_E_HIP;
    }
    if (device_id < 0 || device_id >= ndev) { set_error("tmat_create: bad device id"); return TMAT_E_ARG; }
    TMAT_HIP(hipSetDevice(device_id));
    std::map<std::string, Tensor> m;
    int patch = 0;
    if (!parse_blob(weights_blob, n_bytes, m, patch)) return TMAT_E_WEIGHTS;
    Ctx *c = new Ctx();
    c->device = device_id;
    c->patch = patch;
    c->max_patches = max_patches > 0 ? max_patches : 400;
    if (const char *e = getenv("TMAT_FUSED_SEP")) c->fused_sep = atoi(e) != 0;
    if (const char *e = getenv("TMAT_ROI")) c->roi_on = atoi(e) != 0;
    if (const char *e = getenv("TMAT_ROI_TIGHT")) c->roi_tight = atoi(e) != 0;
    if (const char *e = getenv("TMAT_ROI_EXACT")) c->roi_exact = atoi(e) != 0;
    if (const char *e = getenv("TMAT_ROI_DOWN")) {
        if (strcmp(e, "0") && strcmp(e, "1") && strcmp(e, "2") && strcmp(e, "3")) { set_error("tmat_create: TMAT_ROI_DOWN must be 0, 1, 2 or 3"); delete c; return TMAT_E_ARG; }
        c->roi_down = (unsigned)atoi(e);
    }
    if (const char *e = getenv("TMAT_ROI_CONST")) {
        if (strcmp(e, "0") && strcmp(e, "1")) { set_error("tmat_create: TMAT_ROI_CONST must be 0 or 1"); delete c; return TMAT_E_ARG; }
        c->roi_const = atoi(e);
    }
    if (const char *e = getenv("TMAT_ROI_SHARE")) {
        if (strcmp(e, "0") && strcmp(e, "1")) { set_error("tmat_create: TMAT_ROI_SHARE must be 0 or 1"); delete c; return TMAT_E_ARG; }
        c->roi_share = atoi(e);
    }
    if (const char *e = getenv("TMAT_ROI_SHARE_RECT")) {
        if (strcmp(e, "0") && strcmp(e, "1")) { set_error("tmat_create: TMAT_ROI_SHARE_RECT must be 0 or 1"); delete c; return TMAT_E_ARG; }
        c->roi_share_rect = atoi(e);
    }
    if (const char *e = getenv("TMAT_ROI_SHARE_FUSED_RECT")) {
        if (strcmp(e, "0") && strcmp(e, "1")) { set_error("tmat_create: TMAT_ROI_SHARE_FUSED_RECT must be 0 or 1"); delete c; return TMAT_E_ARG; }
        c->roi_share_fused_rect = atoi(e);
    }
    c->const_cap = c->roi_const == 0 ? 0 : std::max(4, c->max_patches / 64);
    if (const char *e = getenv("TMAT_FUSED_POOL")) c->fused_pool = atoi(e) != 0;
    if (const char *e = getenv("TMAT_STEM_FUSED")) c->stem_fused = atoi(e) != 0;
    if (const char *e = getenv("TMAT_SEP_BF16")) c->sep_bf16 = atoi(e) != 0;
    const char *prec_env = getenv("TMAT_PRECISION");
    if (prec_env && strcmp(prec_env, "f32") && strcmp(prec_env, "bf16x3") && strcmp(prec_env, "bf16x6")) {
        set_error("tmat_create: TMAT_PRECISION must be f32, bf16x3 or bf16x6");
        delete c;
        return TMAT_E_ARG;
    }
    { const int rc = resnet_precision_from_env(c); if (rc) { delete c; return rc; } }
    if (const char *e = getenv("TMAT_DMT_DEVICE")) c->dmt_device = atoi(e) != 0;
    if (const char *e = getenv("TMAT_DMT_SWEEP_DEVICE")) c->dmt_sweep_device = atoi(e) != 0;
    if (const char *e = getenv("TMAT_PRE_STREAM")) c->pre_side = atoi(e) != 0;
    if (const char *e = getenv("TMAT_THIN_DEVICE")) c->thin_device = atoi(e) != 0;
    int prio_least = 0, prio_greatest = 0;
    hipDeviceGetStreamPriorityRange(&prio_least, &prio_greatest);
    if (!hip_ok(hipStreamCreateWithPriority(&c->stream, hipStreamDefault, prio_greatest), "hipStreamCreate") || !build_model(c, m)) { tmat_destroy((tmat_handle)c); return TMAT_E_WEIGHTS; }
    const size_t unit = (size_t)(patch / 2) * (patch / 2) * c->f0;
    const size_t sizes[4] = {unit, unit, 2 * unit, 2 * unit};
    const size_t down_cap = (size_t)c->max_patches + c->const_cap;
    auto dev_f32 = [c](size_t bytes, const char *what) { return (float *)c->ws.dev(bytes, what); };
    for (int i = 0; i < 4; i++)
        if (!(c->buf[i] = dev_f32(sizes[i] * down_cap * sizeof(float), "hipMalloc(activations)"))) { tmat_destroy((tmat_handle)c); return TMAT_E_HIP; }
    const size_t usizes[4] = {unit, unit / 4, unit / 2, unit};
    for (int i = 0; i < 4; i++)
        if (!(c->ubuf[i] = dev_f32(usizes[i] * c->max_patches * sizeof(float), "hipMalloc(up buffers)"))) { tmat_destroy((tmat_handle)c); return TMAT_E_HIP; }
    const size_t dsz = (size_t)(patch >> (1 + c->down.size())) * (patch >> (1 + c->down.size())) * c->up[0].cin;
    const size_t dout_bytes = dsz * down_cap * sizeof(float);
    for (int i = 0; i < 2; i++)
        if (!(c->dout[i] = dev_f32(dout_bytes, "hipMalloc(dout)"))) { tmat_destroy((tmat_handle)c); return TMAT_E_HIP; }
    if (const char *e = getenv("TMAT_RELU_COPY")) c->relu_copy = atoi(e) != 0;
    if (c->relu_copy) {
        size_t need[2] = {0, 0};
        for (size_t j = 0; j + 1 < c->up.size(); j++) {
            const size_t side = (size_t)(patch >> (1 + c->down.size())) << j;
            need[j & 1] = std::max(need[j & 1], side * side * c->up[j].cout);
        }
        for (int i = 0; i < 2; i++)
            if (!(c->dout_relu[i] = dev_f32(dout_bytes, "hipMalloc(dout_relu)")) ||
                (need[i] && !(c->urelu[i] = dev_f32(need[i] * c->max_patches * sizeof(float), "hipMalloc(urelu)")))) { tmat_destroy((tmat_handle)c); return TMAT_E_HIP; }
    }
    if (!hip_ok(hipStreamCreate(&c->stream2), "hipStreamCreate(2)") || !hip_ok(hipStreamCreateWithPriority(&c->stream3, hipStreamDefault, prio_least), "hipStreamCreate(3)")) {
        tmat_destroy((tmat_handle)c); return TMAT_E_HIP;
    }
    for (int i = 0; i < 2; i++)
        if (!hip_ok(hipEventCreateWithFlags(&c->ev_down[i], hipEventDisableTiming), "hipEventCreate") ||
            !hip_ok(hipEventCreateWithFlags(&c->ev_up[i], hipEventDisableTiming), "hipEventCreate") ||
            !hip_ok(hipEventCreateWithFlags(&c->ev_pre[i], hipEventDisableTiming), "hipEventCreate") ||
            !hip_ok(hipEventCreateWithFlags(&c->ev_blend[i], hipEventDisableTiming), "hipEventCreate")) { tmat_destroy((tmat_handle)c); return TMAT_E_HIP; }
    const size_t pp = (size_t)patch * patch * c->max_patches * sizeof(float);
    c->scratch_bytes = 64 << 20;
// ... 180 lines not shown
            float *dev = nullptr;
            if (!upload(c, split_bf16(kv.second.w, mode + 1), &dev)) return TMAT_E_HIP;
            mp[kv.first] = dev;
        }
    }
    { const int rc = tmat_sync(h); if (rc) return rc; }
    c->precision = mode;
    return TMAT_OK;
}

static std::vector<WsEnt> held_blocks(const Ctx *c)
{
    std::vector<WsEnt> all(c->ws.begin(), c->ws.end());
    all.insert(all.end(), c->pass.ws.begin(), c->pass.ws.end());
    for (int i = 0; i < N_TOOL_WS; i++) if (c->tool_ws[i]) all.push_back({c->tool_ws[i], c->tool_ws_bytes[i], false});
    for (auto &b : c->ws_pool) all.push_back({b.second, b.first, false});
    all.insert(all.end(), c->stack_host.begin(), c->stack_host.end());
    return all;
}

int tmat_debug_poison(tmat_handle h, int byte_pattern)
{
    Ctx *c = (Ctx *)h;
    if (!c) { set_error("null handle"); return TMAT_E_ARG; }
    TMAT_HIP(hipSetDevice(c->device));
    { const int rc = tmat_sync(h); if (rc) return rc; }
    std::vector<WsEnt> all = held_blocks(c);
    for (const WsEnt &e : all) {
        if (e.host) memset(e.p, byte_pattern, e.bytes);
        else TMAT_HIP(hipMemsetAsync(e.p, byte_pattern, e.bytes, c->stream));
    }
    TMAT_HIP(hipStreamSynchronize(c->stream));
    return TMAT_OK;
}

int tmat_debug_held_bytes(tmat_handle h, size_t *device_bytes, size_t *pinned_bytes)
{
    Ctx *c = (Ctx *)h;
    if (!c || !device_bytes || !pinned_bytes) { set_error("tmat_debug_held_bytes: bad argument"); return TMAT_E_ARG; }
    *device_bytes = *pinned_bytes = 0;
    for (const WsEnt &e : held_blocks(c)) *(e.host ? pinned_bytes : device_bytes) += e.bytes;
    return TMAT_OK;
}

int tmat_debug_sep_tiles(tmat_handle h, int cap, int *n, long long *planned, long long *full)
{
    Ctx *c = (Ctx *)h;
    if (!c || !n || cap < 0 || (cap > 0 && (!planned || !full))) { set_error("tmat_debug_sep_tiles: bad argument"); return TMAT_E_ARG; }
    *n = (int)c->sep_tiles.size();
    for (int i = 0; i < *n && i < cap; i++) { planned[i] = c->sep_tiles[i].first; full[i] = c->sep_tiles[i].second; }
    return TMAT_OK;
}

int tmat_debug_down_segs(tmat_handle h, int *max_segs)
{
    Ctx *c = (Ctx *)h;
    if (!c || !max_segs) { set_error("tmat_debug_down_segs: bad argument"); return TMAT_E_ARG; }
    *max_segs = c->down_segs;
    return TMAT_OK;
}

int tmat_debug_down_seg_total(tmat_handle h, int *total)
{
    Ctx *c = (Ctx *)h;
    if (!c || !total) { set_error("tmat_debug_down_seg_total: bad argument"); return TMAT_E_ARG; }
    *total = c->down_seg_total;
    return TMAT_OK;
}

static int conv2d_roi_impl(tmat_handle hd, const float *x, int n, int hh, int ww, int cin, const float *w, int ksize, int stride, int subpixel, int cout,
                           const float *scale, const float *shift, const float *resid, int rs, int relu_in, int relu_out, const int *segs, int nseg,
                           float *out, float *out_relu)
{
    Ctx *c = (Ctx *)hd;
    if (!c || !x || !w || !shift || !out || n < 1 || hh < 1 || ww < 1 || cin < 1 || cout < 1 || (ksize != 1 && ksize != 3) || (subpixel && ksize != 3) ||
        (subpixel && (resid || out_relu)) || (rs != 0 && rs != 1) || (rs && ((hh | ww) & 1)) || nseg < 0 || nseg > ROI_MAX_SEGS || (nseg && !segs) ||
        (stride != 1 && (stride != 2 || ksize != 1 || subpixel || resid || ((hh | ww) & 1)))) {
        set_error("tmat_conv2d_roi: bad argument (ksize 1 or 3, sub-pixel form of a 3x3 without residual or activated copy, rs 0 or 1, stride 2 with the "
                  "1x1 form without residual on even sides only, at most 64 segments)");
        return TMAT_E_ARG;
    }
    TMAT_HIP(hipSetDevice(c->device));
    hipStream_t s = c->stream;
    const int up = subpixel ? 2 : 1;
    const size_t nx = (size_t)n * hh * ww * cin, no = (size_t)n * (hh * up / stride) * (ww * up / stride) * cout, nr = (size_t)n * (hh >> rs) * (ww >> rs) * cout;
    DevScope mem(c->ws_pool, s);
    std::vector<float> wk = subpixel ? k_contiguous(subpixel_weights(std::vector<float>(w, w + (size_t)9 * cin * cout), cin, cout).data(), 16, cin, cout)
                                     : k_contiguous(w, ksize * ksize, cin, cout);
    const size_t nw = wk.size();
    const float *hw = mem.keep(std::move(wk));
    float *dx = mem.alloc_from(x, nx), *dw = mem.alloc_from(hw, nw);
    float *dsh = mem.alloc_from(shift, cout), *dsc = scale ? mem.alloc_from(scale, cout) : nullptr;
    float *dr = resid ? mem.alloc_from(resid, nr) : nullptr, *dout = mem.alloc_from((const float *)out, no);
    float *dout2 = out_relu ? mem.alloc_from((const float *)out_relu, no) : nullptr;
    if (!mem.ok) return TMAT_E_HIP;
    ConvArgs a{};
    a.in = dx; a.N = n; a.h = hh; a.w = ww; a.Cin = cin; a.relu_in = relu_in != 0; a.ksize = subpixel ? 2 : ksize; a.stride = stride; a.W = dw;
    a.Cout = cout; a.scale = dsc; a.shift = dsh; a.resid = dr; a.rs = rs; a.relu_out = relu_out != 0; a.out = dout; a.out_relu = dout2; a.prec = 0;
    RoiSegs sg{};
    for (int i = 0; i < nseg; i++) {
        RoiSeg &g = sg.s[sg.nseg++];
        g.p0 = segs[6 * i]; g.np = segs[6 * i + 1]; g.y0 = segs[6 * i + 2]; g.x0 = segs[6 * i + 3]; g.rh = segs[6 * i + 4]; g.rw = segs[6 * i + 5];
    }
    if (!launch_conv(a, s, nseg ? &sg : nullptr)) return TMAT_E_ARG;
    mem.check(hipGetLastError(), "tmat_conv2d_roi launch");
    mem.d2h(out, dout, no * sizeof(float));
// ... 146 lines not shown
```

### tissue-model-analysis-tools_amd/csrc/tmat_ctx.h

```cpp
#pragma once
#include "tmat_internal.h"
#include "dev_mem.h"
#include "gauss_tables.h"
#include "roi_plan.h"

#include <map>

namespace tmat {

struct DownBlock {
    int cin = 0, cout = 0;
    float *dw[2] = {nullptr, nullptr};
    float *pw[2] = {nullptr, nullptr};
    float *scale[2] = {nullptr, nullptr}, *shift[2] = {nullptr, nullptr};
    float *res_w = nullptr, *res_b = nullptr;
};
struct UpBlock {
    int cin = 0, cout = 0;
    float *ct[2] = {nullptr, nullptr};
    float *ct_sub = nullptr;
    float *scale[2] = {nullptr, nullptr}, *shift[2] = {nullptr, nullptr};
    float *res_w = nullptr, *res_b = nullptr;
};
struct ProfEv { hipEvent_t e0, e1; double flops; };
struct RoiTileTab { int layer = 0, k = 0, n = 0; long long full = 0; int *dev = nullptr; RoiDownForm form = ROI_DOWN_REGION; long long n_rep = 0, full_rep = 0; };
struct RoiShareTab {
    int k = 0;
    RoiDownForm form = ROI_DOWN_SHARE;
    std::vector<int> nbr;
    int *nbr_dev = nullptr;
    struct Layer { int layer = 0; std::vector<ShareItem> items; ShareItem *dev = nullptr; };
    std::vector<Layer> layers;
};
struct RoiEntry {
    RoiPlan plan;
    int4 *order = nullptr;
    std::vector<RoiTileTab> tabs;
    std::vector<RoiShareTab> shares;
    void free_tabs()
    {
        for (RoiTileTab &t : tabs) if (t.dev) hipFree(t.dev);
        tabs.clear();
        for (RoiShareTab &t : shares) {
            if (t.nbr_dev) hipFree(t.nbr_dev);
            for (RoiShareTab::Layer &l : t.layers) if (l.dev) hipFree(l.dev);
        }
        shares.clear();
    }
};
struct ConvWHost { std::vector<float> w; int cin; };

struct PassBuf {
    int K = 0, H = 0, W = 0, h = 0, w = 0;
    int *xi = nullptr, *yi = nullptr;
    float *xc = nullptr, *yc = nullptr;
    float *tmp = nullptr, *x = nullptr;
    uint16_t *small = nullptr;
    int *mn = nullptr, *mx = nullptr;
    double *pred[2] = {nullptr, nullptr};
    double *pred_host[2] = {nullptr, nullptr};
    void *morph_ws = nullptr;
    uint8_t *filt[2] = {nullptr, nullptr};
    double *dist[2] = {nullptr, nullptr};
    uint8_t *filt_host[2] = {nullptr, nullptr};
    double *dist_host[2] = {nullptr, nullptr};
    int *conv_host[2] = {nullptr, nullptr};
    int fh = 0, fw = 0;
    void *finish_ws = nullptr;
    uint8_t *skel[2] = {nullptr, nullptr};
    uint8_t *skel_host[2] = {nullptr, nullptr};
    float *field[2] = {nullptr, nullptr}, *f255[2] = {nullptr, nullptr};
    float *f255_host[2] = {nullptr, nullptr};
    void *thin_ws = nullptr;
    int *nfg[2] = {nullptr, nullptr};
    int *nfg_host[2] = {nullptr, nullptr};
    uint32_t *tie = nullptr;
    uint32_t *tie_host[2] = {nullptr, nullptr};
    void *dmt_ws = nullptr;
// ... 70 lines not shown
    bool dout_relu_ok[2] = {false, false};
    float *urelu[2] = {nullptr, nullptr};
    hipStream_t stream2 = nullptr;
    hipStream_t stream3 = nullptr;
    hipEvent_t ev_down[2] = {nullptr, nullptr};
    hipEvent_t ev_pre[2] = {nullptr, nullptr};
    bool down_pending[2] = {false, false};
    hipEvent_t ev_up[2] = {nullptr, nullptr}, ev_blend[2] = {nullptr, nullptr};
    bool blend_pending[2] = {false, false};
    float *patch_in = nullptr, *patch_out = nullptr;
    float *patch_in2 = nullptr;
    bool pre_side = true;
    float input_sat = 65535.f;
    int patch_cap = 0;
    void *scratch = nullptr;
    size_t scratch_bytes = 0;
    WsList ws;
    double *win1d = nullptr;
    std::vector<double> win_host;
    PassBuf pass;
    void free_pass()
    {
        PassBuf &b = pass;
        b.ws.free_all();
        void *lanczos[] = {b.xi, b.yi, b.xc, b.yc};
        for (void *p : lanczos) if (p) hipFree(p);
        for (hipEvent_t e : b.done) if (e) hipEventDestroy(e);
        pass = PassBuf();
    }
    bool thin_device = true;
    uint32_t *ma_table = nullptr;
    double *se_table = nullptr;
    int se_iters = 0;
    bool dmt_device = true;
    bool dmt_sweep_device = true;
    bool fused_pool = true;
    bool norm_on = false;
    float norm_mean = 0.f, norm_std = 1.f;
    int resnet_precision = 0;
    int precision = 0;
    std::map<const float *, ConvWHost> conv_w_host;
    std::map<int, std::map<const float *, float *>> wsplit;
    bool sep_bf16 = true;
    bool stem_fused = true;
    bool roi_on = true;
    bool roi_tight = true;
    bool roi_exact = true;
    unsigned roi_down = 3u;
    int roi_const = -1;
    int const_cap = 0;
    int roi_share = -1;
    int roi_share_rect = -1;
    int roi_share_fused_rect = -1;
    float *padval[2] = {nullptr, nullptr};
    std::vector<RoiEntry *> roi_cache;
    std::vector<std::pair<long long, long long>> sep_tiles;
    int down_segs = 0;
    int down_seg_total = 0;
    bool fused_sep = true;
    void *tool_ws[N_TOOL_WS] = {};
    size_t tool_ws_bytes[N_TOOL_WS] = {};
    WsPool ws_pool;
    WsList stack_host;
    std::vector<std::pair<double, double>> stack_trace;
    bool prof_on = false;
    std::vector<ProfEv> ev_open;
    std::vector<hipEvent_t> ev_pool;
    double prof_ms = 0, prof_flops = 0;
    int64_t prof_launches = 0;
};

int unet_forward_dev(Ctx *c, const float *X, int n, float *Y, hipStream_t s);
int ensure_patch_io(Ctx *c, int n_patches);
RoiDownForm roi_down_resolve(const Ctx *c, const RoiPlan *plan, int kimg, bool have_padval, bool by_default);
int unet_down_dev(Ctx *c, const float *X, int n, float *dout, hipStream_t s, const RoiPlan *plan = nullptr, const float *padval = nullptr,
                  RoiDownForm form = ROI_DOWN_FULL);
int unet_up_dev(Ctx *c, const float *dout, int n, float *Y, hipStream_t s, const RoiPlan *plan = nullptr);
const RoiPlan *roi_attach(Ctx *c, TileGeom &g);
const RoiPlan *roi_find(const Ctx *c, const TileGeom &g);
int predict_smooth_dev(Ctx *c, float *x_dev, int n, int hh, int ww, double *pred_dev);

inline double numpy_pairwise_sum(const double *a, long n)
{
    if (n < 8) {
        double res = 0.0;
        for (long i = 0; i < n; i++) res += a[i];
        return res;
    }
    if (n <= 128) {
        double r[8];
        for (int j = 0; j < 8; j++) r[j] = a[j];
        long i;
        for (i = 8; i < n - (n % 8); i += 8)
            for (int j = 0; j < 8; j++) r[j] += a[i + j];
        double res = ((r[0] + r[1]) + (r[2] + r[3])) + ((r[4] + r[5]) + (r[6] + r[7]));
        for (; i < n; i++) res += a[i];
        return res;
    }
    long n2 = n / 2;
    n2 -= n2 % 8;
    return numpy_pairwise_sum(a, n2) + numpy_pairwise_sum(a + n2, n - n2);
}

inline void *ws_get(Ctx *c, ToolWs slot, size_t bytes)
{
    if (c->tool_ws_bytes[slot] >= bytes && c->tool_ws[slot]) return c->tool_ws[slot];
    if (c->tool_ws[slot]) { hipFree(c->tool_ws[slot]); c->tool_ws[slot] = nullptr; c->tool_ws_bytes[slot] = 0; }
    if (!hip_ok(hipMalloc(&c->tool_ws[slot], bytes ? bytes : 16), "hipMalloc(tool workspace)")) { c->tool_ws[slot] = nullptr; return nullptr; }
    c->tool_ws_bytes[slot] = bytes ? bytes : 16;
    return c->tool_ws[slot];
}

int resnet_precision_from_env(Ctx *c);

inline bool has_model(const Ctx *c) { return c && !c->up.empty(); }
}
```

### tissue-model-analysis-tools_amd/csrc/tmat_internal.h

```cpp
#pragma once
#include <hip/hip_runtime.h>
#include <stdint.h>
#include <string>
#include <vector>

namespace tmat {

void set_error(const std::string &msg);
bool hip_ok(hipError_t e, const char *what);
#define TMAT_HIP(call) do { if (!::tmat::hip_ok((call), #call)) return TMAT_E_HIP; } while (0)

struct ConvArgs {
    const float *in;
    int N, h, w, Cin;
    int relu_in;
    int ksize;
    int stride;
    const float *W;
    int Cout;
    const float *scale;
    const float *shift;
    const float *resid;
    int rs;
    int relu_out;
// ... 46 lines not shown
    q = RoiBox2{0, 0, 0, 0, 0, 0, 0, 0};
    for (int k = 0; k < r.nseg; k++)
        if (n >= r.s[k].p0 && n < r.s[k].p0 + r.s[k].np) {
            const int y0 = r.s[k].y0, y1 = y0 + r.s[k].rh, x0 = r.s[k].x0, x1 = x0 + r.s[k].rw;
            if (!hit) q = RoiBox2{y0, y1, x0, x1, y0, y1, x0, x1};
            if (y0 != q.y0) { q.y2 = y0; q.y3 = y1; }
            if (x0 != q.x0) { q.x2 = x0; q.x3 = x1; }
            hit = true;
        }
    return hit;
}
__device__ __forceinline__ bool roi_box_of(const RoiNone &, int, RoiBox2 &) { return true; }
__device__ __forceinline__ bool roi_box_of(const RoiNone &, int, RoiBox &) { return true; }
#endif
template <class F>
inline int roi_compact_blocks(const RoiSegs &r, int frame_h, int frame_w, int C4, F positions)
{
    long long best = 0, whole = 0;
    for (int i = 0; i < r.nseg;) {
        RoiBox2 q{};
        int j = i;
        for (; j < r.nseg && r.s[j].p0 == r.s[i].p0; j++) {
            const int y0 = r.s[j].y0, y1 = y0 + r.s[j].rh, x0 = r.s[j].x0, x1 = x0 + r.s[j].rw;
            if (j == i) q = RoiBox2{y0, y1, x0, x1, y0, y1, x0, x1};
            if (y0 != q.y0) { q.y2 = y0; q.y3 = y1; }
            if (x0 != q.x0) { q.x2 = x0; q.x3 = x1; }
        }
        const long long n = positions(q);
        if (q.rows() >= frame_h && q.cols() >= frame_w) whole = n; else best = best > n ? best : n;
        i = j;
    }
    if (best == 0) best = whole;
    const long long blocks = (best * C4 + 255) / 256;
    return (int)(blocks < 1 ? 1 : blocks);
}
bool launch_conv(const ConvArgs &a, hipStream_t s, const RoiSegs *roi = nullptr);
struct ConvF16Args {
    const uint16_t *in;
    int N, h, w, Cin;
    int ksize, stride;
    const uint16_t *W;
    int Cout;
    const float *scale;
    const float *shift;
    const uint16_t *resid;
    int relu_out;
    uint16_t *out;
};
bool launch_conv_f16act(const ConvF16Args &a, hipStream_t s);
size_t sepconv_pool_scratch_floats(int N, int H, int W, int Cout);
bool sepconv_ws_supported(int H, int W, int Cin, int Cout);
bool launch_sepconv_ws(const float *in, int N, int H, int W, int Cin, int relu_in, const float *dw9, const float *pwk, int Cout,
                       const float *scale, const float *shift, int relu_out, float *out, hipStream_t s, int prec = 0,
                       const int *tiles = nullptr, int n_tiles = 0);
bool launch_sepconv_pool_ws(const float *in, int N, int H, int W, int Cin, int relu_in, const float *dw9, const float *pwk, int Cout,
                            const float *scale, const float *shift, int relu_out, float *scratch, const float *resid, float *out, hipStream_t s, int prec = 0,
                            const RoiSegs *roi_fix = nullptr,
                            const int *tiles = nullptr, int n_tiles = 0);
void launch_dwconv(const float *in, int N, int H, int W, int C, int relu_in, const float *Wd, float *out, hipStream_t s, const RoiSegs *roi = nullptr);
void launch_stem(const float *x, int N, int H, int W, const float *Ws, int Cout, const float *scale,
                 const float *shift, float *out, hipStream_t s);
void launch_stem_even(const float *x, int N, int H, int W, const float *Ws, int Cout, const float *scale,
                      const float *shift, float *out, hipStream_t s, const RoiSegs *roi = nullptr);
bool launch_sepconv_ws_stem(const float *x, int N, int H, int W, int Cin, const float *stem_w, const float *stem_scale, const float *stem_shift,
                            const float *dw9, const float *pwk, int Cout, const float *scale, const float *shift, int relu_out, float *out,
                            hipStream_t s, const int *tiles = nullptr, int n_tiles = 0);
void launch_maxpool_add(const float *p2, int N, int H, int W, int C, const float *r, float *out, hipStream_t s, float *out_relu = nullptr,
                        const RoiSegs *roi = nullptr);
void launch_final(const float *S, int N, int h, int w, int C, const float *Wf, float bias, float *out, hipStream_t s, const RoiSegs *roi = nullptr);

struct FillItem { int p0, np, cnt, y0, x0, rh, rw; };
struct FillItems { int n; FillItem it[64]; };
bool launch_const_fill(float *t, int src0, int N, int H, int C, const FillItems &f, hipStream_t s);
struct ShareItem { int p0, np, dir, y0, x0, rh, rw; };
bool share_fill_check(int N, int H, int C, const int *nbr, const ShareItem *it, int n);
bool launch_share_fill(float *t, int N, int H, int C, const int *nbr_host, const int *nbr_dev, const ShareItem *it_host, const ShareItem *it_dev, int n,
                       hipStream_t s);
void launch_const_patches(const float *padval, int k, int pp, float *out, hipStream_t s);

struct TileGeom {
    int hh, ww;
    int ws, step, aug;
    int Hp, Wp;
    int na[2], nb[2];
    int tiles_per_img;
    int tile_off[8];
    const int4 *order;
};
TileGeom make_geom(int hh, int ww, int ws);
void launch_minmax_f32(const float *x, int n, size_t per, float *mn, float *mx, hipStream_t s);
void launch_norm_f32(float *x, size_t n, float mean, float sd, hipStream_t s);
void launch_extract_tiles(const float *x, const float *padval, int n, const TileGeom &g, float *patches, hipStream_t s);
void launch_blend(const float *pred_patches, const double *win1d, int n, const TileGeom &g, double *out, hipStream_t s);

bool thin_dev_supported(int H, int W);
size_t thin_workspace_bytes(int n, int H, int W);
int thin_count_dev(const uint8_t *mask, int n, int H, int W, int *nfg, hipStream_t s);
int thin_dev(const uint8_t *mask, const double *dist, const uint32_t *tie, const int *nfg, int n, int H, int W, void *ws,
             const uint32_t *table_dev, uint8_t *skel, hipStream_t s);

inline size_t dmt_edge_count(int R, int C) { return (size_t)(R - 1) * C + (size_t)R * (C - 1) + (size_t)(R - 1) * (C - 1); }
size_t dmt_workspace_bytes(int n, int R, int C);
int dmt_sorted_edges_dev(const float *field, int n, int R, int C, void *ws, int32_t *ids, int *m, hipStream_t s);
size_t dmt_sweep_workspace_bytes(int n, int R, int C);
int dmt_sweeps_dev(const float *field, const int32_t *ids, const int *m, int n, int R, int C, void *ws, uint8_t *kind, float *pers, hipStream_t s);

}
```

### tissue-model-analysis-tools_amd/tmat_amd/_lib.py

```python
from __future__ import annotations

import ctypes as C
import os
from pathlib import Path

import numpy as np

_HERE = Path(__file__).resolve().parent
LIB_PATH = Path(os.environ.get("TMAT_HIP_LIB", _HERE / "libtmat_hip.so"))

_lib = None


class TmatError(RuntimeError):
    pass


E_ARG = -1
E_CAP = -4


class Row(C.Structure):
    _fields_ = [("index", C.c_int64), ("count", C.c_int64), ("total_px", C.c_double), ("avg_px", C.c_double)]

# ... 119 lines not shown
    L.tmat_stack_well_front_dev.argtypes = [vp, vp, i, i, i, i, i, i, vp, vp, vp]
    L.tmat_superellipse_table.argtypes = [vp, vp, i]
    L.tmat_superellipse_search.argtypes = [vp, vp, vp, i, vp, vp, vp, i, C.POINTER(i)]
    L.tmat_superellipse_masks.argtypes = [vp, vp, i, vp, vp, vp, i, i, vp, vp, i, C.POINTER(i)]
    L.tmat_resize_nearest_u8.argtypes = [vp, vp, i, i, i, i, i, vp]
    L.tmat_analyze_batch_masked.argtypes = [vp, vp, i, i, i, C.c_double, i, f, f, i, i, i, i, C.c_int64, vp, vp, vp]
    L.tmat_analyze_batch_ex.argtypes = [vp, vp, i, i, i, C.POINTER(AnalyzeOpts), vp]
    L.tmat_analyze_batch_ex_dev.argtypes = [vp, vp, i, i, i, C.POINTER(AnalyzeOpts), vp]
    L.tmat_analyze_batch_grid.argtypes = [vp, vp, i, i, i, C.POINTER(AnalyzeOpts), C.POINTER(GridOpts), vp]
    L.tmat_analyze_batch_grid_dev.argtypes = [vp, vp, i, i, i, C.POINTER(AnalyzeOpts), C.POINTER(GridOpts), vp]
    L.tmat_render_barcode.argtypes = [vp, vp, vp, i, i, vp]
    L.tmat_render_barcode_png.argtypes = [vp, vp, vp, i, i, vp, sz, vp]
    L.tmat_host_barcode_rects.argtypes = [vp, i, i, vp, i, C.POINTER(i)]
    L.tmat_stage_pictures.argtypes = [vp, vp, i, i, sz, vp]
    L.tmat_host_stage_pictures.argtypes = [vp, i, i, sz, vp]
    L.tmat_png_stripe.argtypes = []
    L.tmat_png_bound.argtypes = [i, i, i, C.POINTER(sz)]
    L.tmat_png_encode_batch.argtypes = [vp, vp, i, i, i, i, vp, sz, vp]
    L.tmat_png_encode_batch_dev.argtypes = L.tmat_png_encode_batch.argtypes
    L.tmat_png_encode_batch_timed.argtypes = L.tmat_png_encode_batch.argtypes + [vp]
    L.tmat_host_png_encode_batch.argtypes = [vp, i, i, i, i, vp, sz, vp]
    L.tmat_render_tree_png.argtypes = [vp, vp, i, i, i, i, vp, vp, vp, i, vp, sz, vp]
    L.tmat_prof_read.argtypes = [vp, C.POINTER(C.c_double), C.POINTER(C.c_int64), C.POINTER(C.c_double), i]
    for name in EXPORTS:
        fn = getattr(L, name)
        if name not in ("tmat_last_error", "tmat_destroy"):
            fn.restype = i
    _lib = L
    return L


EXPORTS = [
    "tmat_last_error", "tmat_version", "tmat_create", "tmat_create_plain", "tmat_destroy", "tmat_sync", "tmat_set_input_depth", "tmat_unet_predict",
    "tmat_predict_smooth", "tmat_segment_batch", "tmat_postprocess_batch", "tmat_filter_edt_batch", "tmat_medial_axis_batch", "tmat_finish_batch", "tmat_filter_mask_batch", "tmat_zproj_batch", "tmat_zproj_dev", "tmat_gather_rows",
    "tmat_dmt_graph", "tmat_dmt_graph_batch", "tmat_morse_stats",
    "tmat_morse_tree", "tmat_branch_color", "tmat_render_tree", "tmat_render_tree_timed", "tmat_host_render_tree", "tmat_host_render_barcode",
    "tmat_analyze_batch_dev", "tmat_analyze_batch", "tmat_analyze_batch_tree_dev", "tmat_analyze_batch_tree", "tmat_dev_alloc", "tmat_dev_free", "tmat_dev_upload", "tmat_dev_download",
    "tmat_prof_enable", "tmat_prof_read", "tmat_debug_poison", "tmat_debug_held_bytes", "tmat_debug_filter_stages", "tmat_set_precision", "tmat_set_input_norm", "tmat_preprocess_batch", "tmat_well_threshold", "tmat_well_threshold_f64", "tmat_canny_mask", "tmat_superellipse_table", "tmat_superellipse_search",
    "tmat_superellipse_masks", "tmat_resize_nearest_u8", "tmat_analyze_batch_masked", "tmat_host_lanczos4_u16", "tmat_host_rescale01_u16",
    "tmat_host_rescale255_f32", "tmat_host_filter_mask", "tmat_host_skeletonize", "tmat_host_medial_axis",
    "tmat_host_permutation", "tmat_host_postprocess",
    "tmat_set_gaussian_table", "tmat_host_gaussian_kernel1d", "tmat_gaussian_f32", "tmat_sato_batch", "tmat_stack_prepare", "tmat_vessel_field",
    "tmat_analyze_stack", "tmat_field_stats", "tmat_field_stats_pruned", "tmat_resize_aa_u16", "tmat_cell_area_batch", "tmat_cell_area_masked", "tmat_resize_linear_u16",
    "tmat_resnet_load", "tmat_resnet_predict", "tmat_inv_depth_predict", "tmat_inv_depth_predict_multi", "tmat_resnet_set_precision", "tmat_conv2d",
    "tmat_roi_plan", "tmat_roi_plan_tight", "tmat_roi_plan_exact", "tmat_conv2d_roi", "tmat_conv2d_roi_s2", "tmat_roi_plan_down", "tmat_roi_sep_tiles", "tmat_debug_sep_tiles", "tmat_debug_down_segs", "tmat_debug_down_seg_total",
    "tmat_roi_plan_const", "tmat_roi_sep_tiles_live", "tmat_roi_plan_share", "tmat_roi_sep_tiles_share", "tmat_roi_plan_share_rect", "tmat_roi_plan_share_fused_rect", "tmat_roi_down_schedule", "tmat_debug_share_fill_check",
    "tmat_stage_pictures", "tmat_host_stage_pictures", "tmat_analyze_batch_ex", "tmat_analyze_batch_ex_dev",
    "tmat_png_stripe", "tmat_png_bound", "tmat_png_encode_batch", "tmat_png_encode_batch_dev", "tmat_png_encode_batch_timed",
    "tmat_host_png_encode_batch", "tmat_render_tree_png",
    "tmat_analyze_stack_batch", "tmat_vessel_field_batch", "tmat_stack_pass_plan", "tmat_debug_stack_trace",
    "tmat_analyze_batch_grid", "tmat_analyze_batch_grid_dev", "tmat_render_barcode", "tmat_render_barcode_png", "tmat_host_barcode_rects",
    "tmat_analyze_stack_batch_dev", "tmat_canny_mask_batch", "tmat_well_small_shape", "tmat_stack_well_front_dev",
    "tmat_cell_small_dev", "tmat_cell_well_front_dev", "tmat_cell_area_fit_dev",
]


def check(rc: int, what: str = ""):
    if rc != 0:
        msg = lib().tmat_last_error()
        raise TmatError(f"{what} failed ({rc}): {msg.decode() if msg else ''}")


def ptr(a: np.ndarray):
    return a.ctypes.data_as(C.c_void_p)


class VesselStages(C.Structure):
    _fields_ = [(k, C.c_void_p) for k in ("vess", "sharp", "vessels", "edges", "skel", "mask_sel", "grown", "closed", "filt")]


class Handle:

    def __init__(self, weights_blob: "bytes | None", device_id: int = 0, max_patches: int = 0):
        L = lib()
        self._h = C.c_void_p()
        self._blob = weights_blob
        if weights_blob is None:
            check(L.tmat_create_plain(device_id, C.byref(self._h)), "tmat_create_plain")
            return
        buf = (C.c_char * len(weights_blob)).from_buffer_copy(weights_blob)
        check(L.tmat_create(device_id, C.cast(buf, C.c_void_p), len(weights_blob), max_patches, C.byref(self._h)),
              "tmat_create")

    @property
    def raw(self):
        return self._h

    def close(self):
        if getattr(self, "_h", None) is not None and self._h.value:
            lib().tmat_destroy(self._h)
            self._h = C.c_void_p()

    def __del__(self):
        try:
            self.close()
        except Exception:
            pass

    def unet_predict(self, x: np.ndarray) -> np.ndarray:
        x = np.ascontiguousarray(x, np.float32)
        y = np.empty_like(x)
        check(lib().tmat_unet_predict(self._h, ptr(x), x.shape[0], ptr(y)), "tmat_unet_predict")
        return y

    def predict_smooth(self, x: np.ndarray) -> np.ndarray:
        x = np.ascontiguousarray(x, np.float32)
# ... 160 lines not shown
        return out, dict(zip(("upload", "minmax", "render", "copy_back"), (float(v) for v in ms)))

    def stage_pictures(self, a):
        a, shape = _stage_pictures_arg(a)
        out = np.empty(a.shape, np.uint8)
        if a.shape[0]:
            check(lib().tmat_stage_pictures(self._h, ptr(a), PIC_DTYPES[a.dtype], a.shape[0], a[0].size, ptr(out)), "tmat_stage_pictures")
        return out.reshape(shape)

    def png_encode(self, pics):
        pics = _png_arg(pics)
        return _png_call(lambda *a: lib().tmat_png_encode_batch(self._h, *a), pics, "tmat_png_encode_batch")

    def png_encode_dev(self, pics_dev, n, H, W, channels):
        return _png_call(lambda _, *a: lib().tmat_png_encode_batch_dev(self._h, pics_dev, *a), (n, H, W, channels), "tmat_png_encode_batch_dev")

    def png_encode_timed(self, pics):
        pics = _png_arg(pics)
        ms = np.zeros(3, np.float32)
        files = _png_call(lambda *a: lib().tmat_png_encode_batch_timed(self._h, *a, ptr(ms)), pics, "tmat_png_encode_batch_timed")
        return files, dict(zip(("upload", "kernels", "copy_back"), (float(v) for v in ms)))

    def render_tree_png(self, backgrounds, trees, vis_width=2000):
        bg, dt, segs, sb, off, _ = _render_tree_args(backgrounds, trees, vis_width, want_out=False)
        vh, vw = tree_canvas_shape(bg.shape[1], bg.shape[2], vis_width)
        return _png_call(lambda _, n, H, W, ch, *a: lib().tmat_render_tree_png(self._h, ptr(bg), dt, n, bg.shape[1], bg.shape[2], ptr(segs), ptr(sb),
                                                                                ptr(off), int(vis_width), *a),
                         (bg.shape[0], vh, vw, 3), "tmat_render_tree_png")

    def render_barcode(self, bars_list, vis_width=2000):
        bars, off = _barcode_args(bars_list)
        S = int(round(vis_width * 0.9))
        out = np.empty((len(bars_list), S, S, 3), np.uint8)
        check(lib().tmat_render_barcode(self._h, ptr(bars), ptr(off), len(bars_list), int(vis_width), ptr(out)), "tmat_render_barcode")
        return out

    def render_barcode_png(self, bars_list, vis_width=2000):
        bars, off = _barcode_args(bars_list)
        S = int(round(vis_width * 0.9))
        return _png_call(lambda _, n, H, W, ch, *a: lib().tmat_render_barcode_png(self._h, ptr(bars), ptr(off), n, int(vis_width), *a),
                         (len(bars_list), S, S, 3), "tmat_render_barcode_png")

    def debug_poison(self, byte_pattern=0xFF):
        check(lib().tmat_debug_poison(self._h, int(byte_pattern)), "tmat_debug_poison")

    def debug_sep_tiles(self):
        L = lib()
        L.tmat_debug_sep_tiles.argtypes = [C.c_void_p, C.c_int, C.c_void_p, C.c_void_p, C.c_void_p]
        n = np.zeros(1, np.int32)
        planned, full = np.zeros(16, np.int64), np.zeros(16, np.int64)
        check(L.tmat_debug_sep_tiles(self._h, 16, ptr(n), ptr(planned), ptr(full)), "tmat_debug_sep_tiles")
        return [(int(planned[i]), int(full[i])) for i in range(min(int(n[0]), 16))]

    def debug_down_segs(self):
        n = C.c_int()
        check(lib().tmat_debug_down_segs(self._h, C.byref(n)), "tmat_debug_down_segs")
        return n.value

    def debug_down_seg_total(self):
        n = C.c_int()
        check(lib().tmat_debug_down_seg_total(self._h, C.byref(n)), "tmat_debug_down_seg_total")
        return n.value

    def debug_held_bytes(self):
        dev, pin = C.c_size_t(), C.c_size_t()
        check(lib().tmat_debug_held_bytes(self._h, C.byref(dev), C.byref(pin)), "tmat_debug_held_bytes")
        return dev.value, pin.value

    def prof_enable(self, on=True):
        check(lib().tmat_prof_enable(self._h, int(on)), "tmat_prof_enable")

    def prof_read(self, reset=True):
        ms, n, fl = C.c_double(), C.c_int64(), C.c_double()
        check(lib().tmat_prof_read(self._h, C.byref(ms), C.byref(n), C.byref(fl), int(reset)), "tmat_prof_read")
        return ms.value, n.value, fl.value


def dmt_graph(img: np.ndarray, delta1: float, delta2: float = 0.0, handle: "Handle | None" = None):
    img = np.ascontiguousarray(img, np.float32)
    R, Cc = img.shape
    cap_v, cap_e = R * Cc + 4, 3 * R * Cc + 4
    V = np.empty((cap_v, 2), np.int32)
    E = np.empty((cap_e, 2), np.int32)
    nv, ne = C.c_int(), C.c_int()
    check(lib().tmat_dmt_graph(handle.raw if handle else None, ptr(img), R, Cc, float(delta1), float(delta2), ptr(V), cap_v,
                               ptr(E), cap_e, C.byref(nv), C.byref(ne)), "tmat_dmt_graph")
    return V[: nv.value].copy(), E[: ne.value].copy()


def dmt_graph_batch(imgs: np.ndarray, delta1: float, delta2: float = 0.0, handle: "Handle | None" = None):
    imgs = np.ascontiguousarray(imgs, np.float32)
    n, R, Cc = imgs.shape
    cap_v, cap_e = R * Cc + 4, 3 * R * Cc + 4
    V = np.empty((n, cap_v, 2), np.int32)
    E = np.empty((n, cap_e, 2), np.int32)
    nv, ne = np.zeros(n, np.int32), np.zeros(n, np.int32)
    check(lib().tmat_dmt_graph_batch(handle.raw if handle else None, ptr(imgs), n, R, Cc, float(delta1), float(delta2), ptr(V), cap_v,
                                     ptr(E), cap_e, ptr(nv), ptr(ne)), "tmat_dmt_graph_batch")
    return [(V[k, : nv[k]].copy(), E[k, : ne[k]].copy()) for k in range(n)]


def morse_stats(V, E, shape, smoothing_window, min_branch_length, max_branch_length=None,
                remove_isolated_branches=False, pruning_mask=None):
    V = np.ascontiguousarray(V, np.int32).reshape(-1, 2)
    E = np.ascontiguousarray(E, np.int32).reshape(-1, 2)
    pm = None
# ... 248 lines not shown
          "roi_plan_share_rect")
    return dict(n_classes=int(ncls[0]), share=share, n_rects=nrect, rects=rects, comp=comp, fills=fills[:int(nfill[0])], mac_rect=mac,
                bytes_rect=byt, any=bool(info[0]), level=int(info[1]), max_segs=int(info[2]))


def roi_plan_share_fused_rect(hh, ww, patch=320, channels=(512, 512, 256, 128, 64), down_channels=(64, 128, 256, 512), fused_mask=3, max_classes=16):
    L = lib()
    L.tmat_roi_plan_share_fused_rect.argtypes = ([C.c_int] * 4 + [C.c_void_p, C.c_int, C.c_void_p, C.c_uint, C.c_int] + [C.c_void_p] * 4 +
                                                 [C.c_int] + [C.c_void_p] * 5)
    n_up, n_down = len(channels) - 1, len(down_channels) - 1
    ch, dch = np.asarray(channels, np.int32), np.asarray(down_channels, np.int32)
    nl = 6 * n_down + 4
    ncls, nfill, info = np.zeros(1, np.int32), np.zeros(1, np.int32), np.zeros(3, np.int32)
    nrect = np.zeros((nl, max_classes), np.int32)
    rects = np.zeros((nl, max_classes, 4, 4), np.int32)
    comp = np.zeros((nl, max_classes, 2, patch), np.uint8)
    cap = nl * max_classes * 12
    fills = np.zeros((cap, 7), np.int32)
    on = np.zeros(nl, np.int32)
    tot = np.zeros((nl, 6), np.float64)
    check(L.tmat_roi_plan_share_fused_rect(hh, ww, patch, n_up, ptr(ch), n_down, ptr(dch), int(fused_mask), max_classes, ptr(ncls), ptr(nrect),
                                           ptr(rects), ptr(comp), cap, ptr(nfill), ptr(fills), ptr(on), ptr(tot), ptr(info)),
          "roi_plan_share_fused_rect")
    return dict(n_classes=int(ncls[0]), n_rects=nrect, rects=rects, comp=comp, fills=fills[:int(nfill[0])], fill_on=on, mac=tot[:, 0],
                bytes=tot[:, 1], px=tot[:, 2], px_live=tot[:, 3], copy_old=tot[:, 4], copy_new=tot[:, 5], any=bool(info[0]),
                levels=int(info[1]), max_segs=int(info[2]))


ROI_DOWN_FORMS = ("full", "region", "const", "share", "share_rect", "share_fused_rect")


def roi_down_schedule(hh, ww, form, k, patch=320, channels=(512, 512, 256, 128, 64), down_channels=(64, 128, 256, 512), fused_mask=3):
    L = lib()
    L.tmat_roi_down_schedule.argtypes = ([C.c_int] * 4 + [C.c_void_p, C.c_int, C.c_void_p, C.c_uint, C.c_int, C.c_int] + [C.c_void_p] * 3 +
                                         [C.c_int, C.c_void_p, C.c_void_p] * 2)
    n_up, n_down = len(channels) - 1, len(down_channels) - 1
    ch, dch = np.asarray(channels, np.int32), np.asarray(down_channels, np.int32)
    nl = 6 * n_down + 4
    info, nseg, ncf, ncp = np.zeros(4, np.int32), np.zeros(nl, np.int32), np.zeros(1, np.int32), np.zeros(1, np.int32)
    segs = np.zeros((nl, 64, 6), np.int32)
    cap = nl * 16 * 12
    cfill, copies = np.zeros((cap, 7), np.int32), np.zeros((cap, 8), np.int32)
    f = ROI_DOWN_FORMS.index(form) if isinstance(form, str) else int(form)
    check(L.tmat_roi_down_schedule(hh, ww, patch, n_up, ptr(ch), n_down, ptr(dch), int(fused_mask), f, int(k), ptr(info), ptr(nseg), ptr(segs),
                                   cap, ptr(ncf), ptr(cfill), cap, ptr(ncp), ptr(copies)), "roi_down_schedule")
    return dict(form=int(info[0]), stem_layer=int(info[1]), max_segs=int(info[2]), seg_total=int(info[3]),
                segs=[segs[l, :int(nseg[l])].copy() for l in range(nl)], const_fills=cfill[:int(ncf[0])], copies=copies[:int(ncp[0])])


def roi_sep_tiles_share(hh, ww, layer, k, patch=320, channels=(512, 512, 256, 128, 64), down_channels=(64, 128, 256, 512), fused_mask=3):
    return roi_sep_tiles(hh, ww, layer, k, patch, channels, down_channels, fused_mask, _export="tmat_roi_sep_tiles_share")


def debug_share_fill_check(n_patches, side, channels, neighbours, items):
    L = lib()
    L.tmat_debug_share_fill_check.argtypes = [C.c_int] * 3 + [C.c_void_p, C.c_int, C.c_void_p]
    nb = np.ascontiguousarray(neighbours, np.int32).reshape(-1, 3)
    it = np.ascontiguousarray(items, np.int32).reshape(-1, 7)
    rc = L.tmat_debug_share_fill_check(int(n_patches), int(side), int(channels), ptr(nb), len(it), ptr(it))
    return None if rc == 0 else L.tmat_last_error().decode()


def roi_sep_tiles(hh, ww, layer, k, patch=320, channels=(512, 512, 256, 128, 64), down_channels=(64, 128, 256, 512), fused_mask=3,
                  _export="tmat_roi_sep_tiles"):
    L = lib()
    fn = getattr(L, _export)
    fn.argtypes = [C.c_int] * 4 + [C.c_void_p, C.c_int, C.c_void_p, C.c_uint] + [C.c_int] * 3 + [C.c_void_p] * 3
    n_up, n_down = len(channels) - 1, len(down_channels) - 1
    ch, dch = np.asarray(channels, np.int32), np.asarray(down_channels, np.int32)
    nt, nf = np.zeros(1, np.int32), np.zeros(1, np.int32)
    args = (hh, ww, patch, n_up, ptr(ch), n_down, ptr(dch), int(fused_mask), int(layer), int(k))
    check(fn(*args, 0, ptr(nt), ptr(nf), None), _export[5:])
    ids = np.zeros(max(int(nt[0]), 1), np.int32)
    check(fn(*args, len(ids), ptr(nt), ptr(nf), ptr(ids)), _export[5:])
    return ids[:int(nt[0])], int(nf[0])


def host_lanczos4_u16(img, out_hw):
    img = np.ascontiguousarray(img, np.uint16)
    out = np.empty(out_hw, np.uint16)
    L = lib()
    L.tmat_host_lanczos4_u16.argtypes = [C.c_void_p, C.c_int, C.c_int, C.c_int, C.c_int, C.c_void_p]
    check(L.tmat_host_lanczos4_u16(ptr(img), img.shape[0], img.shape[1], out_hw[0], out_hw[1], ptr(out)), "lanczos4")
    return out


def host_rescale01_u16(img):
    img = np.ascontiguousarray(img, np.uint16)
    out = np.empty(img.shape, np.float32)
    L = lib()
    L.tmat_host_rescale01_u16.argtypes = [C.c_void_p, C.c_size_t, C.c_void_p]
    check(L.tmat_host_rescale01_u16(ptr(img), img.size, ptr(out)), "rescale01")
    return out


def host_rescale255_f32(img):
    img = np.ascontiguousarray(img, np.float32)
    out = np.empty(img.shape, np.float32)
    L = lib()
    L.tmat_host_rescale255_f32.argtypes = [C.c_void_p, C.c_size_t, C.c_void_p]
    check(L.tmat_host_rescale255_f32(ptr(img), img.size, ptr(out)), "rescale255")
    return out


def host_filter_mask(mask, use_median=True, remove_isolated=True):
    m = np.ascontiguousarray(np.asarray(mask) != 0, np.uint8)
# ... 42 lines not shown
```

Before: 51.44 images/s.

## Schedule separable-conv ROI work at 8x8 quad granularity instead of 16x16 tiles

Adds a quad table that splits each live 16x16 ROI tile into four 8x8 quads and keeps only the quads whose rows and columns hold live pixels. The workspace sepconv kernel gains a QUAD mode in which each work item covers four quads, with store addresses computed per quad. It is enabled by default in the down pass. The aim is to skip more dead pixels at the edges of the region, in exchange for more table reads, split stores and weaker spatial locality per work item.

```diff
diff --git a/include/tmat.h b/include/tmat.h
--- a/include/tmat.h
+++ b/include/tmat.h
@@ -364,6 +364,11 @@
                            unsigned fused_mask, int form, int k, int *info, int *n_segs, int *segs, int const_cap, int *n_const,
                            int *const_fills, int copy_cap, int *n_copy, int *copies);
 int tmat_debug_share_fill_check(int n_patches, int side, int channels, const int *neighbours, int n_items, const int *items);
+int tmat_roi_sep_quads(int hh, int ww, int patch, int n_up, const int *up_channels, int n_down, const int *down_channels,
+                       unsigned fused_mask, int form, int layer, int k, int cap, int *counts, int *ids);
+int tmat_debug_sepconv_quads(tmat_handle h, const float *x, int n, int hh, int ww, int cin, int relu_in, const float *dw9, const float *pw,
+                             int cout, const float *scale, const float *shift, int relu_out, const float *stem_w, const float *stem_scale,
+                             const float *stem_shift, const int *quads, int n_quads, float *out);
 
 int tmat_debug_sep_tiles(tmat_handle h, int cap, int *n, long long *planned, long long *full);
 int tmat_debug_down_segs(tmat_handle h, int *max_segs);
diff --git a/tissue-model-analysis-tools_amd/csrc/pipeline.cpp b/tissue-model-analysis-tools_amd/csrc/pipeline.cpp
--- a/tissue-model-analysis-tools_amd/csrc/pipeline.cpp
+++ b/tissue-model-analysis-tools_amd/csrc/pipeline.cpp
@@ -144,7 +144,7 @@
     const RoiPlan *plan = roi_find(c, g);
     int rc = oversize ? unet_forward_dev(c, pin, k * g.tiles_per_img, c->patch_out, s)
                       : unet_down_dev(c, pin, k * g.tiles_per_img, c->dout[slot], s, plan, c->padval[slot],
-                                      roi_down_resolve(c, plan, k, c->padval[slot] != nullptr, true));
+                                      roi_down_resolve(c, plan, k, c->padval[slot] != nullptr, true), roi_quad_on(c, true));
     if (rc) return rc;
     TMAT_HIP(hipEventRecord(c->ev_down[slot], s));
     c->down_pending[slot] = true;
diff --git a/tissue-model-analysis-tools_amd/csrc/roi_plan.cpp b/tissue-model-analysis-tools_amd/csrc/roi_plan.cpp
--- a/tissue-model-analysis-tools_amd/csrc/roi_plan.cpp
+++ b/tissue-model-analysis-tools_amd/csrc/roi_plan.cpp
@@ -774,6 +774,40 @@
     return full;
 }
 
+long long roi_sep_quad_table(const RoiPlan &p, RoiDownForm form, int layer, int k, std::vector<int> &out, long long *n_own, long long *n_ids)
+{
+    out.clear();
+    *n_own = *n_ids = 0;
+    const RoiDownPlan &d = p.down;
+    if (form < ROI_DOWN_SHARE || roi_down_form(p, form) < ROI_DOWN_CONST || layer < 0 || layer % 6 != 1 || d.comp.empty()) return 0;
+    form = roi_down_form(p, form);
+    std::vector<int> tiles;
+    const long long full = roi_sep_tile_table(p, form, layer, k, tiles);
+    if (full <= 0) return 0;
+    const int TW = d.res[layer] / 16, TPP = TW * TW, QW = 2 * TW, QPP = QW * QW;
+    if (((long long)k * p.tiles_per_img + k) * QPP > 0x7fffffffLL) return 0;
+    std::vector<int> cls_of((size_t)k * p.tiles_per_img, 0);
+    for (int cl = 0; cl < p.n_classes; cl++)
+        for (int pt = k * p.class_base[cl]; pt < k * p.class_base[cl + 1]; pt++) cls_of[pt] = cl;
+    auto holds = [&](int cl, int axis, int q) {
+        const unsigned char *m = d.comp.data() + (((size_t)layer * ROI_MAX_CLASSES + cl) * 2 + axis) * p.ws + 8 * q;
+        return std::any_of(m, m + 8, [](unsigned char v) { return v != 0; });
+    };
+    for (int id : tiles) {
+        const int pt = id / TPP, tr = id % TPP, ty = tr / TW, tx = tr % TW, cl = cls_of[pt];
+        for (int qy = 2 * ty; qy < 2 * ty + 2; qy++)
+            for (int qx = 2 * tx; qx < 2 * tx + 2; qx++)
+                if (holds(cl, 0, qy) && holds(cl, 1, qx)) out.push_back(pt * QPP + qy * QW + qx);
+    }
+    *n_own = (long long)out.size();
+    for (int pt = k * p.tiles_per_img; pt < k * p.tiles_per_img + k; pt++)
+        for (int tr = 0; tr < TPP; tr++)
+            for (int s = 0; s < 4; s++) out.push_back(pt * QPP + (2 * (tr / TW) + (s >> 1)) * QW + 2 * (tr % TW) + (s & 1));
+    *n_ids = (long long)out.size();
+    while (out.size() % 4) out.push_back(out.back());
+    return full;
+}
+
 void roi_down_segs(const RoiPlan &p, RoiDownForm form, int l, int k, RoiSegs &out)
 {
     out = RoiSegs{};
@@ -1063,6 +1097,24 @@
     return sep_tiles_export(ROI_DOWN_SHARE, hh, ww, patch, n_up, up_channels, n_down, down_channels, fused_mask, layer, k, cap, n_tiles, n_full, tiles);
 }
 
+extern "C" int tmat_roi_sep_quads(int hh, int ww, int patch, int n_up, const int *up_channels, int n_down, const int *down_channels,
+                                  unsigned fused_mask, int form, int layer, int k, int cap, int *counts, int *ids)
+{
+    RoiPlan p;
+    if (int rc = down_plan_for("tmat_roi_sep_quads", counts && k >= 1 && form >= ROI_DOWN_FULL && form <= ROI_DOWN_SHARE_FUSED_RECT, hh, ww, patch, n_up,
+                               up_channels, n_down, down_channels, fused_mask, ROI_MAX_CLASSES, p)) return rc;
+    std::vector<int> tab;
+    long long n_own = 0, n_ids = 0;
+    const long long full = roi_sep_quad_table(p, (RoiDownForm)form, layer, k, tab, &n_own, &n_ids);
+    if (full <= 0) { set_error("tmat_roi_sep_quads: not a plain fused layer of the plan under a sharing form"); return TMAT_E_ARG; }
+    counts[0] = (int)tab.size(); counts[1] = (int)n_own; counts[2] = (int)n_ids; counts[3] = (int)full;
+    if (ids) {
+        if ((int)tab.size() > cap) { set_error("tmat_roi_sep_quads: cap too small"); return TMAT_E_ARG; }
+        std::copy(tab.begin(), tab.end(), ids);
+    }
+    return TMAT_OK;
+}
+
 extern "C" int tmat_roi_plan_const(int hh, int ww, int patch, int n_up, const int *up_channels, int n_down, const int *down_channels,
                                    unsigned fused_mask, int max_classes, int *n_classes, int *nonconst, int *live, int *rect_live, int *fill,
                                    int *stored, double *mac_live, double *bytes_live)
diff --git a/tissue-model-analysis-tools_amd/csrc/roi_plan.h b/tissue-model-analysis-tools_amd/csrc/roi_plan.h
--- a/tissue-model-analysis-tools_amd/csrc/roi_plan.h
+++ b/tissue-model-analysis-tools_amd/csrc/roi_plan.h
@@ -62,6 +62,7 @@
 constexpr unsigned ROI_SHARE_LEVELS = 3u;
 constexpr unsigned ROI_SHARE_RECT_LEVELS = 4u;
 constexpr unsigned ROI_SHARE_FUSED_RECT_LEVELS = 3u;
+constexpr unsigned ROI_QUAD_LEVELS = 3u;
 
 struct RoiPlan {
     int hh = 0, ww = 0, ws = 0, n_up = 0;
@@ -92,6 +93,7 @@
 int roi_down_rects(const RoiPlan &p, RoiDownForm form, int l, int k, RoiRect out[4]);
 int roi_down_stem_layer(const RoiPlan &p, RoiDownForm form);
 long long roi_sep_tile_table(const RoiPlan &p, RoiDownForm form, int layer, int k, std::vector<int> &out);
+long long roi_sep_quad_table(const RoiPlan &p, RoiDownForm form, int layer, int k, std::vector<int> &out, long long *n_own, long long *n_ids);
 void roi_down_segs(const RoiPlan &p, RoiDownForm form, int l, int k, RoiSegs &out);
 void roi_down_const_items(const RoiPlan &p, RoiDownForm form, int l, int k, FillItems &out);
 void roi_down_copy_items(const RoiPlan &p, RoiDownForm form, int l, int k, std::vector<ShareItem> &out);
diff --git a/tissue-model-analysis-tools_amd/csrc/sepconv_ws_kernels.hip b/tissue-model-analysis-tools_amd/csrc/sepconv_ws_kernels.hip
--- a/tissue-model-analysis-tools_amd/csrc/sepconv_ws_kernels.hip
+++ b/tissue-model-analysis-tools_amd/csrc/sepconv_ws_kernels.hip
@@ -58,10 +58,11 @@
     return *((const __attribute__((address_space(4))) int *)(unsigned long long)tab + mt);
 }
 
-template <bool RELU_IN, bool POOL, int PREC = 0, bool STEM = false, bool ROI = false>
+template <bool RELU_IN, bool POOL, int PREC = 0, bool STEM = false, bool ROI = false, bool QUAD = false>
 __global__ __launch_bounds__(768, 3) void sepconv_ws_kernel(WsArgs a, int nMt, int nNt, int G, std::conditional_t<ROI, const int *, RoiNone> tab)
 {
     static_assert(!ROI || PREC == 0, "ROI: f32 path only");
+    static_assert(!QUAD || (ROI && !POOL && PREC == 0), "QUAD: plain region form of the f32 path only");
     __shared__ __attribute__((aligned(16))) float smem[STEM ? WS_TOTAL_STEM : WS_TOTAL];
 
     const int b = blockIdx.x;
@@ -72,7 +73,7 @@
 
     const int t = threadIdx.x;
     const int lane = t & 63, wave = __builtin_amdgcn_readfirstlane(t >> 6);
-    const int TW = a.W >> 4, TPP = (a.H >> 4) * TW;
+    const int TW = QUAD ? a.W >> 3 : a.W >> 4, TPP = QUAD ? (a.H >> 3) * TW : (a.H >> 4) * TW;
     const int Cin = a.Cin;
     const int nchunks = Cin >> 5;
     const int total = (j1 - j0) * nchunks;
@@ -128,12 +129,12 @@
             }
         }
         const float *hA = a.in;
-        int tnext = ws_tab_read(j0 / nNt, tab);
+        int tnext = ws_tab_read(QUAD ? 4 * (j0 / nNt) + p : j0 / nNt, tab);
         auto tile_setup = [&](int jj) {
             const int mt = ROI ? tnext : jj / nNt;
-            if (ROI) tnext = ws_tab_read((jj + 1 < j1 ? jj + 1 : jj) / nNt, tab);
+            if (ROI) { const int mn = (jj + 1 < j1 ? jj + 1 : jj) / nNt; tnext = ws_tab_read(QUAD ? 4 * mn + p : mn, tab); }
             const int n = mt / TPP, tr = mt - n * TPP;
-            const int Y0 = (tr / TW) * 16 + oy - 1, X0 = (tr % TW) * 16 + ox - 1;
+            const int Y0 = QUAD ? (tr / TW) * 8 - 1 : (tr / TW) * 16 + oy - 1, X0 = QUAD ? (tr % TW) * 8 - 1 : (tr % TW) * 16 + ox - 1;
             const unsigned bad = m_inv | (Y0 < 0 ? m_top : 0u) | (Y0 + 9 >= a.H ? m_bot : 0u) | (X0 < 0 ? m_left : 0u) | (X0 + 9 >= a.W ? m_right : 0u);
             if (STEM) {
                 hA = a.in + ((long)n * a.H * a.W * 4 + (long)(2 * Y0) * (2 * a.W) + 2 * X0);
@@ -389,7 +390,9 @@
     const float relu_lo = a.relu_out ? 0.f : -__builtin_inff();
     const unsigned vo_pool = (unsigned)(4 * h * a.Cout + r) * 4u;
     float rv[4][4];
-    int ctile = ws_tab_read(j0 / nNt, tab);
+    const int cslot = 2 * (wave >> 2);
+    int ctile = ws_tab_read(QUAD ? 4 * (j0 / nNt) + cslot : j0 / nNt, tab);
+    int ctile1 = QUAD ? ws_tab_read(4 * (j0 / nNt) + cslot + 1, tab) : 0;
     auto load_resid = [&](int jj) {
         const int mc = jj / nNt, nt = jj - mc * nNt;
         const int mt = ROI ? ctile : mc;
@@ -410,15 +413,19 @@
 #pragma unroll
     for (int i = 0; i < 4; i++) {
         const int pix = 8 * i + (lane >> 3);
-        vo_t[i] = (unsigned)(((pix >> 4) * a.W + (pix & 15)) * a.Cout + (lane & 7) * 4) * 4u;
+        vo_t[i] = (unsigned)(((pix >> 4) * a.W + (QUAD ? pix & 7 : pix & 15)) * a.Cout + (lane & 7) * 4) * 4u;
     }
     auto store_tile = [&](int jj, float *xw) {
         const int mc = jj / nNt, nt = jj - mc * nNt;
         const int mt = ROI ? ctile : mc;
         const int n = mt / TPP, tr = mt - n * TPP;
-        const int ty0 = (tr / TW) * 16, tx0 = (tr % TW) * 16;
+        const int ty0 = QUAD ? (tr / TW) * 8 : (tr / TW) * 16, tx0 = QUAD ? (tr % TW) * 8 : (tr % TW) * 16;
+        const int trow = QUAD ? 2 * (wave & 3) : 2 * wave;
         const __amdgpu_buffer_rsrc_t rsO = __builtin_amdgcn_make_buffer_rsrc(
-            (void *)(a.out + ((size_t)n * a.H * a.W + (size_t)(ty0 + 2 * wave) * a.W + tx0) * a.Cout + nt * 128), 0, 0x7fffffff, 0x00020000);
+            (void *)(a.out + ((size_t)n * a.H * a.W + (size_t)(ty0 + trow) * a.W + tx0) * a.Cout + nt * 128), 0, 0x7fffffff, 0x00020000);
+        const int n1 = ctile1 / TPP, tr1 = ctile1 - n1 * TPP;
+        const __amdgpu_buffer_rsrc_t rsO1 = !QUAD ? rsO : __builtin_amdgcn_make_buffer_rsrc(
+            (void *)(a.out + ((size_t)n1 * a.H * a.W + (size_t)((tr1 / TW) * 8 + trow) * a.W + (tr1 % TW) * 8) * a.Cout + nt * 128), 0, 0x7fffffff, 0x00020000);
         float *xl = xw + r;
         const float *xr = xw + lane * 4;
 #pragma unroll
@@ -435,7 +442,7 @@
             for (int i = 0; i < 4; i++) o[i] = *reinterpret_cast<const float4 *>(xr + i * 256);
 #pragma unroll
             for (int i = 0; i < 4; i++)
-                __builtin_amdgcn_raw_buffer_store_b128(__builtin_bit_cast(__attribute__((ext_vector_type(4))) unsigned, o[i]), rsO, vo_t[i], jn * 128, 0);
+                __builtin_amdgcn_raw_buffer_store_b128(__builtin_bit_cast(__attribute__((ext_vector_type(4))) unsigned, o[i]), (i & 1) ? rsO1 : rsO, vo_t[i], jn * 128, 0);
         }
     };
 
@@ -649,7 +656,10 @@
             if (POOL) store_tile_pool(cj, smem + (stage ? WS_A : 0));
             else store_tile(cj, smem + (stage ? WS_A1 : WS_A0) + wave * 1024);
             cj++;
-            if (ROI && s + 1 < total) ctile = ws_tab_read(cj / nNt, tab);
+            if (ROI && s + 1 < total) {
+                ctile = ws_tab_read(QUAD ? 4 * (cj / nNt) + cslot : cj / nNt, tab);
+                if (QUAD) ctile1 = ws_tab_read(4 * (cj / nNt) + cslot + 1, tab);
+            }
         }
         WS_PIN()
         if (s + 1 < total) {
@@ -690,9 +700,11 @@
            (long long)H * W * Cin * 4 < 0x7fffffffLL && (long long)Cout * Cin * 4 < 0x7fffffffLL;
 }
 
-static bool ws_tiles_ok(const int *tiles, int n_tiles, int N, int H, int W, int prec)
-{
-    return !tiles || (prec == 0 && n_tiles > 0 && (long long)n_tiles <= (long long)N * (H / 16) * (W / 16));
+static bool ws_tiles_ok(const int *tiles, int n_tiles, int N, int H, int W, int prec, bool quad = false)
+{
+    if (!tiles) return !quad;
+    if (quad) return prec == 0 && n_tiles > 0 && n_tiles <= 0x0fffffff;
+    return prec == 0 && n_tiles > 0 && (long long)n_tiles <= (long long)N * (H / 16) * (W / 16);
 }
 
 static int ws_cus()
@@ -708,10 +720,17 @@
 }
 
 template <bool POOL>
-static void launch_ws_any(const WsArgs &a, int relu_in, int prec, hipStream_t s, const int *tiles = nullptr, int n_tiles = 0)
+static void launch_ws_any(const WsArgs &a, int relu_in, int prec, hipStream_t s, const int *tiles = nullptr, int n_tiles = 0, bool quad = false)
 {
     const int nMt = tiles ? n_tiles : a.N * (a.H / 16) * (a.W / 16), nNt = a.Cout / 128;
     const int G = (ws_cus() / 8) * 8;
+    if constexpr (!POOL) {
+        if (quad && tiles && prec == 0) {
+            if (relu_in) hipLaunchKernelGGL((sepconv_ws_kernel<true, false, 0, false, true, true>), dim3(G), dim3(768), 0, s, a, nMt, nNt, G, tiles);
+            else hipLaunchKernelGGL((sepconv_ws_kernel<false, false, 0, false, true, true>), dim3(G), dim3(768), 0, s, a, nMt, nNt, G, tiles);
+            return;
+        }
+    }
     if (prec == 1) {
         if (relu_in) hipLaunchKernelGGL((sepconv_ws_kernel<true, POOL, 1>), dim3(G), dim3(768), 0, s, a, nMt, nNt, G, RoiNone{});
         else hipLaunchKernelGGL((sepconv_ws_kernel<false, POOL, 1>), dim3(G), dim3(768), 0, s, a, nMt, nNt, G, RoiNone{});
@@ -750,31 +769,32 @@
 }
 
 bool launch_sepconv_ws(const float *in, int N, int H, int W, int Cin, int relu_in, const float *dw9, const float *pwk, int Cout,
-                       const float *scale, const float *shift, int relu_out, float *out, hipStream_t s, int prec, const int *tiles, int n_tiles)
+                       const float *scale, const float *shift, int relu_out, float *out, hipStream_t s, int prec, const int *tiles, int n_tiles, bool quad)
 {
     if (!sepconv_ws_supported(H, W, Cin, Cout) || N <= 0 || (long long)N * (H / 16) * (W / 16) * (Cout / 128) > 0x3fffffffLL ||
-        !ws_tiles_ok(tiles, n_tiles, N, H, W, prec)) {
+        !ws_tiles_ok(tiles, n_tiles, N, H, W, prec, quad) || (quad && (long long)n_tiles * (Cout / 128) > 0x3fffffffLL)) {
         set_error("launch_sepconv_ws: unsupported shape");
         return false;
     }
     WsArgs a{in, N, H, W, Cin, Cout, dw9, pwk, scale, shift, relu_out, out, nullptr, nullptr, nullptr, nullptr, nullptr, nullptr, nullptr};
-    launch_ws_any<false>(a, relu_in, prec, s, tiles, n_tiles);
+    launch_ws_any<false>(a, relu_in, prec, s, tiles, n_tiles, quad);
     return true;
 }
 
 bool launch_sepconv_ws_stem(const float *x, int N, int H, int W, int Cin, const float *stem_w, const float *stem_scale, const float *stem_shift,
                             const float *dw9, const float *pwk, int Cout, const float *scale, const float *shift, int relu_out, float *out,
-                            hipStream_t s, const int *tiles, int n_tiles)
+                            hipStream_t s, const int *tiles, int n_tiles, bool quad)
 {
     if (!sepconv_ws_supported(H, W, Cin, Cout) || N <= 0 || (long long)N * (H / 16) * (W / 16) * (Cout / 128) > 0x3fffffffLL || 9 * Cin > WS_X ||
-        !ws_tiles_ok(tiles, n_tiles, N, H, W, 0)) {
+        !ws_tiles_ok(tiles, n_tiles, N, H, W, 0, quad) || (quad && (long long)n_tiles * (Cout / 128) > 0x3fffffffLL)) {
         set_error("launch_sepconv_ws_stem: unsupported shape");
         return false;
     }
     WsArgs a{x, N, H, W, Cin, Cout, dw9, pwk, scale, shift, relu_out, out, nullptr, nullptr, nullptr, nullptr, stem_w, stem_scale, stem_shift};
     const int nMt = tiles ? n_tiles : N * (H / 16) * (W / 16), nNt = Cout / 128;
     const int G = (ws_cus() / 8) * 8;
-    if (tiles) hipLaunchKernelGGL((sepconv_ws_kernel<false, false, 0, true, true>), dim3(G), dim3(768), 0, s, a, nMt, nNt, G, tiles);
+    if (tiles && quad) hipLaunchKernelGGL((sepconv_ws_kernel<false, false, 0, true, true, true>), dim3(G), dim3(768), 0, s, a, nMt, nNt, G, tiles);
+    else if (tiles) hipLaunchKernelGGL((sepconv_ws_kernel<false, false, 0, true, true>), dim3(G), dim3(768), 0, s, a, nMt, nNt, G, tiles);
     else hipLaunchKernelGGL((sepconv_ws_kernel<false, false, 0, true>), dim3(G), dim3(768), 0, s, a, nMt, nNt, G, RoiNone{});
     return true;
 }
diff --git a/tissue-model-analysis-tools_amd/csrc/tmat_api.cpp b/tissue-model-analysis-tools_amd/csrc/tmat_api.cpp
--- a/tissue-model-analysis-tools_amd/csrc/tmat_api.cpp
+++ b/tissue-model-analysis-tools_amd/csrc/tmat_api.cpp
@@ -274,13 +274,27 @@
     return ok;
 }
 
-static const RoiTileTab *roi_tile_tab(RoiEntry *e, int layer, int k, RoiDownForm form)
+static const RoiTileTab *roi_tile_tab(RoiEntry *e, int layer, int k, RoiDownForm form, bool quad = false)
 {
     form = roi_down_form(e->plan, std::min(form, ROI_DOWN_SHARE));
-    for (const RoiTileTab &t : e->tabs) if (t.layer == layer && t.k == k && t.form == form) return &t;
+    for (const RoiTileTab &t : e->tabs) if (t.layer == layer && t.k == k && t.form == form && t.quad == quad) return &t;
     std::vector<int> ids;
     RoiTileTab t;
     t.layer = layer; t.k = k; t.form = form;
+    if (quad) {
+        long long n_own = 0, n_ids = 0;
+        t.full_rep = t.full = roi_sep_quad_table(e->plan, form, layer, k, ids, &n_own, &n_ids);
+        if (t.full > 0) {
+            t.quad = true;
+            t.n = (int)(ids.size() / 4);
+            t.n_rep = (n_own + 3) / 4;
+            if (!hip_ok(hipMalloc((void **)&t.dev, ids.size() * sizeof(int)), "hipMalloc(quadrant table)")) return nullptr;
+            if (!hip_ok(hipMemcpy(t.dev, ids.data(), ids.size() * sizeof(int), hipMemcpyHostToDevice), "hipMemcpy(quadrant table)")) { hipFree(t.dev); return nullptr; }
+            e->tabs.push_back(t);
+            return &e->tabs.back();
+        }
+        return roi_tile_tab(e, layer, k, form);
+    }
     t.full = roi_sep_tile_table(e->plan, form, layer, k, ids);
     t.n_rep = (long long)ids.size(); t.full_rep = t.full;
     if (t.full <= 0 || ids.empty()) { set_error("roi_tile_tab: no tile table for this layer"); return nullptr; }
@@ -368,7 +382,7 @@
     return roi_down_form(*plan, want);
 }
 
-int unet_down_dev(Ctx *c, const float *X, int n, float *dout, hipStream_t s, const RoiPlan *plan, const float *padval, RoiDownForm form)
+int unet_down_dev(Ctx *c, const float *X, int n, float *dout, hipStream_t s, const RoiPlan *plan, const float *padval, RoiDownForm form, bool quad)
 {
     if (n <= 0) return TMAT_OK;
     if (n > c->max_patches) { set_error("unet_down_dev: n > max_patches"); return TMAT_E_ARG; }
@@ -413,7 +427,8 @@
         t.full = t.n = n * (H / 16) * (H / 16);
         t.full_rep = t.n_rep = (long long)n_own * (H / 16) * (H / 16);
         if (ent && f32) {
-            if (const RoiTileTab *made = roi_tile_tab(ent, 6 * (int)bi + k, kimg, form)) t = *made;
+            const bool q = quad && k == 1 && form >= ROI_DOWN_SHARE && ((ROI_QUAD_LEVELS >> bi) & 1u);
+            if (const RoiTileTab *made = roi_tile_tab(ent, 6 * (int)bi + k, kimg, form, q)) t = *made;
             else tab_ok = false;
         }
         c->sep_tiles.push_back({t.dev ? t.n_rep : t.full_rep, t.full_rep});
@@ -445,8 +460,8 @@
             if (!tab_ok) return TMAT_E_HIP;
             if (stem_here) {
                 if (!launch_sepconv_ws_stem(X, n, H, H, d.cin, c->stem_w, c->stem_scale, c->stem_shift, d.dw[0], pw0, d.cout, d.scale[0], d.shift[0], 1, b2, s,
-                                            t0.dev, t0.n)) return TMAT_E_ARG;
-            } else if (!launch_sepconv_ws(b0, n, H, H, d.cin, bi > 0, d.dw[0], pw0, d.cout, d.scale[0], d.shift[0], 1, b2, s, sprec, t0.dev, t0.n)) return TMAT_E_ARG;
+                                            t0.dev, t0.n, t0.quad)) return TMAT_E_ARG;
+            } else if (!launch_sepconv_ws(b0, n, H, H, d.cin, bi > 0, d.dw[0], pw0, d.cout, d.scale[0], d.shift[0], 1, b2, s, sprec, t0.dev, t0.n, t0.quad)) return TMAT_E_ARG;
             if (!copies(b2, 6 * (int)bi + 1, d.cout)) return TMAT_E_ARG;
             ConvArgs r{};
             r.in = b0; r.N = n; r.h = H; r.w = H; r.Cin = d.cin; r.ksize = 1; r.stride = 2; r.W = d.res_w; r.Cout = d.cout;
@@ -626,7 +641,7 @@
         const float *xi = x_dev + (size_t)i0 * hh * ww;
         launch_minmax_f32(xi, k, (size_t)hh * ww, mn, mx, c->stream);
         launch_extract_tiles(xi, mn, k, g, c->patch_in, c->stream);
-        int rc = plan ? unet_down_dev(c, c->patch_in, k * g.tiles_per_img, c->dout[0], c->stream, plan, mn, roi_down_resolve(c, plan, k, true, false))
+        int rc = plan ? unet_down_dev(c, c->patch_in, k * g.tiles_per_img, c->dout[0], c->stream, plan, mn, roi_down_resolve(c, plan, k, true, false), roi_quad_on(c, false))
                       : unet_forward_dev(c, c->patch_in, k * g.tiles_per_img, c->patch_out, c->stream);
         if (!rc && plan) rc = unet_up_dev(c, c->dout[0], k * g.tiles_per_img, c->patch_out, c->stream, plan);
         if (rc) return rc;
@@ -711,6 +726,10 @@
     if (const char *e = getenv("TMAT_ROI_SHARE_FUSED_RECT")) {
         if (strcmp(e, "0") && strcmp(e, "1")) { set_error("tmat_create: TMAT_ROI_SHARE_FUSED_RECT must be 0 or 1"); delete c; return TMAT_E_ARG; }
         c->roi_share_fused_rect = atoi(e);
+    }
+    if (const char *e = getenv("TMAT_ROI_QUAD")) {
+        if (strcmp(e, "0") && strcmp(e, "1")) { set_error("tmat_create: TMAT_ROI_QUAD must be 0 or 1"); delete c; return TMAT_E_ARG; }
+        c->roi_quad = atoi(e);
     }
     c->const_cap = c->roi_const == 0 ? 0 : std::max(4, c->max_patches / 64);
     if (const char *e = getenv("TMAT_FUSED_POOL")) c->fused_pool = atoi(e) != 0;
@@ -997,6 +1016,46 @@
     return TMAT_OK;
 }
 
+int tmat_debug_sepconv_quads(tmat_handle hd, const float *x, int n, int hh, int ww, int cin, int relu_in, const float *dw9, const float *pw, int cout,
+                             const float *scale, const float *shift, int relu_out, const float *stem_w, const float *stem_scale,
+                             const float *stem_shift, const int *quads, int n_quads, float *out)
+{
+    Ctx *c = (Ctx *)hd;
+    const bool stem = stem_w != nullptr;
+    if (!c || !x || !dw9 || !pw || !scale || !shift || !quads || !out || n < 1 || n_quads < 1 || n_quads > (1 << 24) || hh < 16 || ww < 16 || cin < 1 ||
+        cout < 1 || stem != (stem_scale != nullptr) || stem != (stem_shift != nullptr) || (stem && relu_in) || !sepconv_ws_supported(hh, ww, cin, cout) ||
+        (long long)n * hh * ww * std::max(cin, cout) > 0x3fffffffLL) {
+        set_error("tmat_debug_sepconv_quads: bad argument");
+        return TMAT_E_ARG;
+    }
+    const long long nq = (long long)n * (hh / 8) * (ww / 8);
+    std::vector<int> ids(quads, quads + n_quads);
+    for (int id : ids) if (id < 0 || id >= nq) { set_error("tmat_debug_sepconv_quads: a quadrant id lies outside the tensor"); return TMAT_E_ARG; }
+    while (ids.size() % 4) ids.push_back(ids.back());
+    TMAT_HIP(hipSetDevice(c->device));
+    hipStream_t s = c->stream;
+    DevScope mem(c->ws_pool, s);
+    const size_t nx = stem ? (size_t)n * hh * ww * 4 : (size_t)n * hh * ww * cin, no = (size_t)n * hh * ww * cout;
+    std::vector<float> wk = k_contiguous(pw, 1, cin, cout);
+    const size_t nw = wk.size();
+    const float *hw = mem.keep(std::move(wk));
+    const size_t n_ids = ids.size();
+    const int *hid = mem.keep(std::move(ids));
+    float *dx = mem.alloc_from(x, nx), *dd = mem.alloc_from(dw9, (size_t)9 * cin), *dw = mem.alloc_from(hw, nw);
+    float *dsc = mem.alloc_from(scale, cout), *dsh = mem.alloc_from(shift, cout), *dout = mem.alloc_from((const float *)out, no);
+    float *sw = stem ? mem.alloc_from(stem_w, (size_t)9 * cin) : nullptr, *ssc = stem ? mem.alloc_from(stem_scale, cin) : nullptr;
+    float *ssh = stem ? mem.alloc_from(stem_shift, cin) : nullptr;
+    int *dq = mem.alloc_from(hid, n_ids);
+    if (!mem.ok) return TMAT_E_HIP;
+    const bool ok = stem ? launch_sepconv_ws_stem(dx, n, hh, ww, cin, sw, ssc, ssh, dd, dw, cout, dsc, dsh, relu_out != 0, dout, s, dq, (int)(n_ids / 4), true)
+                         : launch_sepconv_ws(dx, n, hh, ww, cin, relu_in != 0, dd, dw, cout, dsc, dsh, relu_out != 0, dout, s, 0, dq, (int)(n_ids / 4), true);
+    if (!ok) return TMAT_E_ARG;
+    mem.check(hipGetLastError(), "tmat_debug_sepconv_quads launch");
+    mem.d2h(out, dout, no * sizeof(float));
+    if (mem.finish()) return TMAT_E_HIP;
+    return TMAT_OK;
+}
+
 int tmat_debug_down_segs(tmat_handle h, int *max_segs)
 {
     Ctx *c = (Ctx *)h;
diff --git a/tissue-model-analysis-tools_amd/csrc/tmat_ctx.h b/tissue-model-analysis-tools_amd/csrc/tmat_ctx.h
--- a/tissue-model-analysis-tools_amd/csrc/tmat_ctx.h
+++ b/tissue-model-analysis-tools_amd/csrc/tmat_ctx.h
@@ -23,7 +23,10 @@
     float *res_w = nullptr, *res_b = nullptr;
 };
 struct ProfEv { hipEvent_t e0, e1; double flops; };
-struct RoiTileTab { int layer = 0, k = 0, n = 0; long long full = 0; int *dev = nullptr; RoiDownForm form = ROI_DOWN_REGION; long long n_rep = 0, full_rep = 0; };
+struct RoiTileTab {
+    int layer = 0, k = 0, n = 0; long long full = 0; int *dev = nullptr; RoiDownForm form = ROI_DOWN_REGION; long long n_rep = 0, full_rep = 0;
+    bool quad = false;
+};
 struct RoiShareTab {
     int k = 0;
     RoiDownForm form = ROI_DOWN_SHARE;
@@ -200,6 +203,7 @@
     int roi_share = -1;
     int roi_share_rect = -1;
     int roi_share_fused_rect = -1;
+    int roi_quad = -1;
     float *padval[2] = {nullptr, nullptr};
     std::vector<RoiEntry *> roi_cache;
     std::vector<std::pair<long long, long long>> sep_tiles;
@@ -222,7 +226,8 @@
 int ensure_patch_io(Ctx *c, int n_patches);
 RoiDownForm roi_down_resolve(const Ctx *c, const RoiPlan *plan, int kimg, bool have_padval, bool by_default);
 int unet_down_dev(Ctx *c, const float *X, int n, float *dout, hipStream_t s, const RoiPlan *plan = nullptr, const float *padval = nullptr,
-                  RoiDownForm form = ROI_DOWN_FULL);
+                  RoiDownForm form = ROI_DOWN_FULL, bool quad = false);
+inline bool roi_quad_on(const Ctx *c, bool by_default) { return by_default ? c->roi_quad != 0 : c->roi_quad == 1; }
 int unet_up_dev(Ctx *c, const float *dout, int n, float *Y, hipStream_t s, const RoiPlan *plan = nullptr);
 const RoiPlan *roi_attach(Ctx *c, TileGeom &g);
 const RoiPlan *roi_find(const Ctx *c, const TileGeom &g);
diff --git a/tissue-model-analysis-tools_amd/csrc/tmat_internal.h b/tissue-model-analysis-tools_amd/csrc/tmat_internal.h
--- a/tissue-model-analysis-tools_amd/csrc/tmat_internal.h
+++ b/tissue-model-analysis-tools_amd/csrc/tmat_internal.h
@@ -122,7 +122,7 @@
 bool sepconv_ws_supported(int H, int W, int Cin, int Cout);
 bool launch_sepconv_ws(const float *in, int N, int H, int W, int Cin, int relu_in, const float *dw9, const float *pwk, int Cout,
                        const float *scale, const float *shift, int relu_out, float *out, hipStream_t s, int prec = 0,
-                       const int *tiles = nullptr, int n_tiles = 0);
+                       const int *tiles = nullptr, int n_tiles = 0, bool quad = false);
 bool launch_sepconv_pool_ws(const float *in, int N, int H, int W, int Cin, int relu_in, const float *dw9, const float *pwk, int Cout,
                             const float *scale, const float *shift, int relu_out, float *scratch, const float *resid, float *out, hipStream_t s, int prec = 0,
                             const RoiSegs *roi_fix = nullptr,
@@ -134,7 +134,7 @@
                       const float *shift, float *out, hipStream_t s, const RoiSegs *roi = nullptr);
 bool launch_sepconv_ws_stem(const float *x, int N, int H, int W, int Cin, const float *stem_w, const float *stem_scale, const float *stem_shift,
                             const float *dw9, const float *pwk, int Cout, const float *scale, const float *shift, int relu_out, float *out,
-                            hipStream_t s, const int *tiles = nullptr, int n_tiles = 0);
+                            hipStream_t s, const int *tiles = nullptr, int n_tiles = 0, bool quad = false);
 void launch_maxpool_add(const float *p2, int N, int H, int W, int C, const float *r, float *out, hipStream_t s, float *out_relu = nullptr,
                         const RoiSegs *roi = nullptr);
 void launch_final(const float *S, int N, int h, int w, int C, const float *Wf, float bias, float *out, hipStream_t s, const RoiSegs *roi = nullptr);
diff --git a/tissue-model-analysis-tools_amd/tmat_amd/_lib.py b/tissue-model-analysis-tools_amd/tmat_amd/_lib.py
--- a/tissue-model-analysis-tools_amd/tmat_amd/_lib.py
+++ b/tissue-model-analysis-tools_amd/tmat_amd/_lib.py
@@ -195,6 +195,7 @@
     "tmat_analyze_batch_grid", "tmat_analyze_batch_grid_dev", "tmat_render_barcode", "tmat_render_barcode_png", "tmat_host_barcode_rects",
     "tmat_analyze_stack_batch_dev", "tmat_canny_mask_batch", "tmat_well_small_shape", "tmat_stack_well_front_dev",
     "tmat_cell_small_dev", "tmat_cell_well_front_dev", "tmat_cell_area_fit_dev",
+    "tmat_roi_sep_quads", "tmat_debug_sepconv_quads",
 ]
 
 
@@ -461,6 +462,24 @@
         check(L.tmat_debug_sep_tiles(self._h, 16, ptr(n), ptr(planned), ptr(full)), "tmat_debug_sep_tiles")
         return [(int(planned[i]), int(full[i])) for i in range(min(int(n[0]), 16))]
 
+    def debug_sepconv_quads(self, x, dw9, pw, scale, shift, quads, out, relu_in=False, relu_out=True, stem=None):
+        x, dw9, pw = (np.ascontiguousarray(a, np.float32) for a in (x, dw9, pw))
+        scale, shift = np.ascontiguousarray(scale, np.float32), np.ascontiguousarray(shift, np.float32)
+        q = np.ascontiguousarray(quads, np.int32).ravel()
+        cin, cout = pw.shape
+        n, hh, ww = out.shape[:3]
+        assert out.dtype == np.float32 and out.flags.c_contiguous and out.shape == (n, hh, ww, cout) and dw9.shape == (9, cin)
+        assert x.shape == ((n, 2 * hh, 2 * ww) if stem is not None else (n, hh, ww, cin)), x.shape
+        st = [None] * 3 if stem is None else [np.ascontiguousarray(a, np.float32) for a in stem]
+        assert stem is None or (st[0].shape == (9, cin) and st[1].shape == (cin,) and st[2].shape == (cin,))
+        L = lib()
+        vp, i = C.c_void_p, C.c_int
+        L.tmat_debug_sepconv_quads.argtypes = [vp, vp, i, i, i, i, i, vp, vp, i, vp, vp, i, vp, vp, vp, vp, i, vp]
+        check(L.tmat_debug_sepconv_quads(self._h, ptr(x), n, hh, ww, cin, int(bool(relu_in)), ptr(dw9), ptr(pw), cout, ptr(scale), ptr(shift),
+                                         int(bool(relu_out)), *(None if a is None else ptr(a) for a in st), ptr(q), len(q), ptr(out)),
+              "tmat_debug_sepconv_quads")
+        return out
+
     def debug_down_segs(self):
         n = C.c_int()
         check(lib().tmat_debug_down_segs(self._h, C.byref(n)), "tmat_debug_down_segs")
@@ -815,6 +834,20 @@
     return roi_sep_tiles(hh, ww, layer, k, patch, channels, down_channels, fused_mask, _export="tmat_roi_sep_tiles_share")
 
 
+def roi_sep_quads(hh, ww, layer, k, form="share", patch=320, channels=(512, 512, 256, 128, 64), down_channels=(64, 128, 256, 512), fused_mask=3):
+    L = lib()
+    L.tmat_roi_sep_quads.argtypes = [C.c_int] * 4 + [C.c_void_p, C.c_int, C.c_void_p, C.c_uint] + [C.c_int] * 4 + [C.c_void_p] * 2
+    n_up, n_down = len(channels) - 1, len(down_channels) - 1
+    ch, dch = np.asarray(channels, np.int32), np.asarray(down_channels, np.int32)
+    f = ROI_DOWN_FORMS.index(form) if isinstance(form, str) else int(form)
+    counts = np.zeros(4, np.int32)
+    args = (hh, ww, patch, n_up, ptr(ch), n_down, ptr(dch), int(fused_mask), f, int(layer), int(k))
+    check(L.tmat_roi_sep_quads(*args, 0, ptr(counts), None), "roi_sep_quads")
+    ids = np.zeros(max(int(counts[0]), 1), np.int32)
+    check(L.tmat_roi_sep_quads(*args, len(ids), ptr(counts), ptr(ids)), "roi_sep_quads")
+    return ids[:int(counts[0])], int(counts[1]), int(counts[2]), int(counts[3])
+
+
 def debug_share_fill_check(n_patches, side, channels, neighbours, items):
     L = lib()
     L.tmat_debug_share_fill_check.argtypes = [C.c_int] * 3 + [C.c_void_p, C.c_int, C.c_void_p]
```

After: 52.03 images/s (median of 6 runs). +1.1%, better.
